# kanyu369/ADNM-UNet

Measured on AMD Instinct MI355X. Metric: sequences/sec training ADNM-UNet 5->20x128x128, higher is better.
Workload: dtype bf16; 1 GPU; ADNM-UNet create_ADNMUNet(5,20,6) 128x128 full training step (fwd + enRainfallLoss + bwd + clip_grad_norm_ + AdamW), recipe parameters, synthetic radar frames in HBM; per_gpu_batch=4, global_batch=4, frames=5->20, parallelism=single, launch=hipGraph replay

## Files before the change

### adnm-unet_amd/csrc/adnm_common.h

```cpp
#pragma once
#include <hip/hip_runtime.h>
#include <hip/hip_bf16.h>
#include <stdint.h>
#include <stdio.h>
#include <stdarg.h>
#include <string.h>
#include "../../include/adnm_hip.h"

#define ADNM_WAVE 64

void adnm_set_error(const char* fmt, ...);

struct AdnmProfScope {
  AdnmProfScope(const char* name, hipStream_t st, double bytes);
  ~AdnmProfScope();
  hipStream_t st_;
  long idx_;
};
#define ADNM_PROF(name, st, bytes) AdnmProfScope adnm_prof_scope__(name, st, (double)(bytes))

struct AdnmFoldSeg {
  float* ptr;
  int len;
};
void adnm_launch_fold(const char* prof_name, const float* part, int rows, int n, AdnmFoldSeg s0, AdnmFoldSeg s1, AdnmFoldSeg s2,
                      AdnmFoldSeg s3, hipStream_t st);

int64_t adnm_lgemm_ws_bytes(int64_t I, int64_t J, int64_t R, int nbs);
int adnm_lgemm_launch(bool b_oc, const float* a, int64_t lda, const void* b, int64_t ldb, int b_dtype, const float* b_scale, const float* bias, float* c,
                      int64_t ldc, void* ws, int64_t ws_bytes, void* slabs_uc, int64_t slabs_uc_bytes, int64_t I, int64_t J, int64_t R, int nbs, int prec,
                      float* q, const char* prof, double prof_bytes, hipStream_t st);
static inline int64_t adnm_ticket_bytes(int64_t ntiles) { return (ntiles * 4 + 255) / 256 * 256; }

struct AdnmLeaf {
  int kind, grid, prec;
  const char* prof;
  double bytes;
  alignas(16) unsigned char args[200];
};
enum {
  ADNM_LEAF_SKGEMM_TN = 0, ADNM_LEAF_DWCONV_WGRAD_K3 = 1, ADNM_LEAF_DWCONV_WGRAD_K5 = 2, ADNM_LEAF_TSGEMM_TN = 3,
  ADNM_LEAF_DWCONV_WALK3 = 4,
  ADNM_LEAF_CONV3_WGRAD = 5,
  ADNM_LEAF_COLSUM = 6,
  ADNM_LEAF_KINDS = 7
};
bool adnm_leafq_active();
bool adnm_leafq_push(const AdnmLeaf& leaf);
int adnm_skgemm_tn_launch_multi(const AdnmLeaf* const* items, int n, hipStream_t st);
int adnm_dwconv_wgrad_launch_multi(const AdnmLeaf* const* items, int n, int K, hipStream_t st);
int adnm_dwconv_walk3_launch_multi(const AdnmLeaf* const* items, int n, hipStream_t st);
int adnm_conv3_wgrad_launch_multi(const AdnmLeaf* const* items, int n, hipStream_t st);
int adnm_tsgemm_tn_launch_multi(const AdnmLeaf* const* items, int n, hipStream_t st);

constexpr int ADNM_GROUP_MAX = 8;
constexpr int ADNM_GROUP_POS_LAST = 1 << 20;
struct AdnmGroupRec;
typedef int (*AdnmGroupFn)(const AdnmGroupRec* const* recs, int n, hipStream_t st);
struct AdnmGroupRec {
  AdnmGroupFn fn;
  int grid, pos;
  const char* prof;
  double bytes;
  alignas(16) unsigned char args[232];
};
bool adnm_group_open();
void adnm_launch_fold_recorded(const char* prof_name, const float* part, int rows, int n, AdnmFoldSeg s0, AdnmFoldSeg s1, AdnmFoldSeg s2,
                               AdnmFoldSeg s3, hipStream_t st);
int adnm_group_submit(const AdnmGroupRec& rec, hipStream_t st);
template <typename Args>
struct AdnmMulti {
  int blk_end[ADNM_GROUP_MAX];
  Args p[ADNM_GROUP_MAX];
};
template <typename Args>
static inline unsigned adnm_group_pack(const AdnmGroupRec* const* r, int n, AdnmMulti<Args>& m) {
  static_assert(sizeof(Args) <= sizeof(AdnmGroupRec::args), "the argument struct must fit a group record");
  static_assert(sizeof(AdnmMulti<Args>) <= 4096, "the descriptor table must fit the kernel argument segment");
  int blocks = 0;
  for (int k = 0; k < ADNM_GROUP_MAX; ++k) {
    if (k < n) memcpy(&m.p[k], r[k]->args, sizeof(Args)), blocks += r[k]->grid;
    else m.p[k] = m.p[0];
    m.blk_end[k] = blocks;
  }
  return (unsigned)blocks;
}
template <typename M>
__device__ __forceinline__ int adnm_group_which(const M& m, int* bid, int* nblk) {
  int k = 0;
#pragma unroll
  for (int i = 0; i < ADNM_GROUP_MAX - 1; ++i) k += (int)blockIdx.x >= m.blk_end[i] ? 1 : 0;
  const int b0 = k ? m.blk_end[k - 1] : 0;
  *bid = (int)blockIdx.x - b0, *nblk = m.blk_end[k] - b0;
  return k;
}

#define ADNM_REQUIRE(cond, ...)            \
  do {                                     \
    if (!(cond)) {                         \
      adnm_set_error(__VA_ARGS__);         \
      return ADNM_EINVAL;                  \
    }                                      \
  } while (0)

#define ADNM_CHECK_LAUNCH(name)                                              \
  do {                                                                       \
    hipError_t e__ = hipGetLastError();                                      \
    if (e__ != hipSuccess) {                                                 \
      adnm_set_error("%s: launch failed: %s", name, hipGetErrorString(e__)); \
      return ADNM_ELAUNCH;                                                   \
    }                                                                        \
  } while (0)

#include <atomic>
#include <initializer_list>
static inline int adnm_allow_lds(const void* fn, size_t smem, std::atomic<uint64_t>& done, const char* name) {
  if (smem <= 64 * 1024) return ADNM_OK;
  int dev = 0;
  if (hipGetDevice(&dev) != hipSuccess) dev = 0;
  const uint64_t bit = 1ull << (dev & 63);
  if (done.load(std::memory_order_relaxed) & bit) return ADNM_OK;
  const hipError_t e = hipFuncSetAttribute(fn, hipFuncAttributeMaxDynamicSharedMemorySize, 160 * 1024);
  if (e != hipSuccess) {
    adnm_set_error("%s: cannot raise the dynamic LDS limit to %zu bytes on device %d: %s", name, smem, dev, hipGetErrorString(e));
    return ADNM_ELAUNCH;
  }
  done.fetch_or(bit, std::memory_order_relaxed);
  return ADNM_OK;
}
#define ADNM_ALLOW_LDS(kernel, smem, name)                                             \
  do {                                                                                 \
    static std::atomic<uint64_t> lds_done__{0};                                        \
    if (int rc__ = adnm_allow_lds((const void*)(kernel), (smem), lds_done__, name)) return rc__; \
  } while (0)

static inline int64_t adnm_cdiv(int64_t a, int64_t b) { return (a + b - 1) / b; }
static inline bool adnm_quad_aligned(int dtype, std::initializer_list<const void*> ptrs) {
  uintptr_t bits = 0;
  for (const void* p : ptrs) bits |= (uintptr_t)p;
  return bits % (dtype == ADNM_BF16 ? 8 : 16) == 0;
}
static inline int64_t adnm_align(int64_t a, int64_t b) { return adnm_cdiv(a, b) * b; }

struct bf16x4 {
  uint16_t v[4];
};

__device__ __forceinline__ float bf16_to_f32(uint16_t h) { return __uint_as_float(((uint32_t)h) << 16); }
__device__ __forceinline__ uint16_t f32_to_bf16(float f) {
  __hip_bfloat16 b = __float2bfloat16(f);
  return *reinterpret_cast<uint16_t*>(&b);
}

template <typename T>
struct Io;
template <>
struct Io<float> {
  static __device__ __forceinline__ float4 ld4(const float* p) { return *reinterpret_cast<const float4*>(p); }
  static __device__ __forceinline__ void st4(float* p, float4 v) { *reinterpret_cast<float4*>(p) = v; }
  static __device__ __forceinline__ float ld(const float* p) { return *p; }
  static __device__ __forceinline__ void st(float* p, float v) { *p = v; }
  static __device__ __forceinline__ float rt(float v) { return v; }
};
template <>
struct Io<uint16_t> {
  static __device__ __forceinline__ float4 ld4(const uint16_t* p) {
    uint2 r = *reinterpret_cast<const uint2*>(p);
    return make_float4(__uint_as_float(r.x << 16), __uint_as_float(r.x & 0xffff0000u), __uint_as_float(r.y << 16),
                       __uint_as_float(r.y & 0xffff0000u));
  }
  static __device__ __forceinline__ void st4(uint16_t* p, float4 v) {
    uint2 r;
    r.x = (uint32_t)f32_to_bf16(v.x) | ((uint32_t)f32_to_bf16(v.y) << 16);
    r.y = (uint32_t)f32_to_bf16(v.z) | ((uint32_t)f32_to_bf16(v.w) << 16);
    *reinterpret_cast<uint2*>(p) = r;
  }
  static __device__ __forceinline__ float ld(const uint16_t* p) { return bf16_to_f32(*p); }
  static __device__ __forceinline__ void st(uint16_t* p, float v) { *p = f32_to_bf16(v); }
  static __device__ __forceinline__ float rt(float v) { return bf16_to_f32(f32_to_bf16(v)); }
};

template <int BT>
__device__ __forceinline__ float4 adnm_ldb4(const void* base, int64_t off) {
  if constexpr (BT == ADNM_B_BF16) {
    const uint2 r = *reinterpret_cast<const uint2*>(reinterpret_cast<const uint16_t*>(base) + off);
    return make_float4(__uint_as_float(r.x << 16), __uint_as_float(r.x & 0xffff0000u), __uint_as_float(r.y << 16), __uint_as_float(r.y & 0xffff0000u));
  } else if constexpr (BT == ADNM_B_FP8) {
    using f2 = __attribute__((ext_vector_type(2))) float;
    const int r = *reinterpret_cast<const int*>(reinterpret_cast<const uint8_t*>(base) + off);
    const f2 lo = __builtin_amdgcn_cvt_pk_f32_fp8(r, false), hi = __builtin_amdgcn_cvt_pk_f32_fp8(r, true);
    return make_float4(lo[0], lo[1], hi[0], hi[1]);
  } else {
    return *reinterpret_cast<const float4*>(reinterpret_cast<const float*>(base) + off);
  }
}

using adnm_f32x4 = __attribute__((ext_vector_type(4))) float;
using adnm_bf16x8 = __attribute__((ext_vector_type(8))) __bf16;

struct AdnmQuant {
  float scale_a, scale_b, amax_a, amax_b, fmax_a, fmax_b, record, pad;
};

struct AdnmStepStats {
  double applied, skipped, norm_sum, norm_max, last_norm, clip_count, loss_sum, loss_nonfinite;
  int skip;
  float sumsq;
};
__device__ __forceinline__ bool adnm_nonfinite_bits(float v) { return (__float_as_uint(v) & 0x7f800000u) == 0x7f800000u; }

__device__ __forceinline__ adnm_bf16x8 adnm_pack_bf16x8(const float (&v)[8]) {
  using f8 = __attribute__((ext_vector_type(8))) float;
  const f8 t = {v[0], v[1], v[2], v[3], v[4], v[5], v[6], v[7]};
  return __builtin_convertvector(t, adnm_bf16x8);
}
template <bool BF8>
__device__ __forceinline__ long adnm_pack_f8x8(const float (&v)[8]) {
  constexpr float kMax = BF8 ? 57344.f : 448.f;
  float c[8];
#pragma unroll
  for (int i = 0; i < 8; ++i) c[i] = __builtin_amdgcn_fmed3f(v[i], kMax, -kMax);
  int lo = 0, hi = 0;
  if (BF8) {
    lo = __builtin_amdgcn_cvt_pk_bf8_f32(c[0], c[1], lo, false), lo = __builtin_amdgcn_cvt_pk_bf8_f32(c[2], c[3], lo, true);
    hi = __builtin_amdgcn_cvt_pk_bf8_f32(c[4], c[5], hi, false), hi = __builtin_amdgcn_cvt_pk_bf8_f32(c[6], c[7], hi, true);
  } else {
    lo = __builtin_amdgcn_cvt_pk_fp8_f32(c[0], c[1], lo, false), lo = __builtin_amdgcn_cvt_pk_fp8_f32(c[2], c[3], lo, true);
    hi = __builtin_amdgcn_cvt_pk_fp8_f32(c[4], c[5], hi, false), hi = __builtin_amdgcn_cvt_pk_fp8_f32(c[6], c[7], hi, true);
  }
  return (long)(((unsigned long)(unsigned)hi << 32) | (unsigned long)(unsigned)lo);
}
template <int PREC, bool P_BF8 = false, bool Q_BF8 = false>
__device__ __forceinline__ adnm_f32x4 adnm_mfma32(const float (&p)[8], const float (&q)[8], adnm_f32x4 acc) {
  if constexpr (PREC == ADNM_MFMA_BF16) {
    return __builtin_amdgcn_mfma_f32_16x16x32_bf16(adnm_pack_bf16x8(p), adnm_pack_bf16x8(q), acc, 0, 0, 0);
  } else if constexpr (PREC == ADNM_MFMA_FP8) {
    const long a = adnm_pack_f8x8<P_BF8>(p), b = adnm_pack_f8x8<Q_BF8>(q);
    if constexpr (P_BF8 && Q_BF8) return __builtin_amdgcn_mfma_f32_16x16x32_bf8_bf8(a, b, acc, 0, 0, 0);
    else if constexpr (P_BF8) return __builtin_amdgcn_mfma_f32_16x16x32_bf8_fp8(a, b, acc, 0, 0, 0);
    else if constexpr (Q_BF8) return __builtin_amdgcn_mfma_f32_16x16x32_fp8_bf8(a, b, acc, 0, 0, 0);
    else return __builtin_amdgcn_mfma_f32_16x16x32_fp8_fp8(a, b, acc, 0, 0, 0);
  } else {
#pragma unroll
    for (int e = 0; e < 8; ++e) acc = __builtin_amdgcn_mfma_f32_16x16x4f32(p[e], q[e], acc, 0, 0, 0);
    return acc;
  }
}
template <int PREC, bool P_BF8 = false, bool Q_BF8 = false>
__device__ __forceinline__ adnm_f32x4 adnm_mfma16(const float (&p)[4], const float (&q)[4], adnm_f32x4 acc) {
  if constexpr (PREC == ADNM_MFMA_F32) {
#pragma unroll
    for (int e = 0; e < 4; ++e) acc = __builtin_amdgcn_mfma_f32_16x16x4f32(p[e], q[e], acc, 0, 0, 0);
    return acc;
  } else {
    const float p8[8] = {p[0], p[1], p[2], p[3], 0.f, 0.f, 0.f, 0.f}, q8[8] = {q[0], q[1], q[2], q[3], 0.f, 0.f, 0.f, 0.f};
    return adnm_mfma32<PREC, P_BF8, Q_BF8>(p8, q8, acc);
  }
}
template <int PREC>
struct AdnmFrag {
  float v[8];
};
template <>
struct AdnmFrag<ADNM_MFMA_BF16> {
  adnm_bf16x8 v;
};
template <>
struct AdnmFrag<ADNM_MFMA_FP8> {
  long v;
};
template <int PREC, bool BF8>
__device__ __forceinline__ AdnmFrag<PREC> adnm_make_frag(const float (&lo)[4], const float* hi, float scale) {
  AdnmFrag<PREC> f;
  float t[8];
#pragma unroll
  for (int e = 0; e < 4; ++e) t[e] = lo[e], t[4 + e] = hi ? hi[e] : 0.f;
  if constexpr (PREC == ADNM_MFMA_BF16) {
    f.v = adnm_pack_bf16x8(t);
  } else if constexpr (PREC == ADNM_MFMA_FP8) {
#pragma unroll
    for (int e = 0; e < 8; ++e) t[e] *= scale;
    f.v = adnm_pack_f8x8<BF8>(t);
  } else {
#pragma unroll
    for (int e = 0; e < 8; ++e) f.v[e] = t[e];
  }
  return f;
}
template <int PREC, bool P_BF8, bool Q_BF8, bool HALF = false>
__device__ __forceinline__ adnm_f32x4 adnm_mma(const AdnmFrag<PREC>& p, const AdnmFrag<PREC>& q, adnm_f32x4 acc) {
  if constexpr (PREC == ADNM_MFMA_BF16) {
    return __builtin_amdgcn_mfma_f32_16x16x32_bf16(p.v, q.v, acc, 0, 0, 0);
  } else if constexpr (PREC == ADNM_MFMA_FP8) {
    if constexpr (P_BF8 && Q_BF8) return __builtin_amdgcn_mfma_f32_16x16x32_bf8_bf8(p.v, q.v, acc, 0, 0, 0);
    else if constexpr (P_BF8) return __builtin_amdgcn_mfma_f32_16x16x32_bf8_fp8(p.v, q.v, acc, 0, 0, 0);
    else if constexpr (Q_BF8) return __builtin_amdgcn_mfma_f32_16x16x32_fp8_bf8(p.v, q.v, acc, 0, 0, 0);
    else return __builtin_amdgcn_mfma_f32_16x16x32_fp8_fp8(p.v, q.v, acc, 0, 0, 0);
  } else {
#pragma unroll
    for (int e = 0; e < (HALF ? 4 : 8); ++e) acc = __builtin_amdgcn_mfma_f32_16x16x4f32(p.v[e], q.v[e], acc, 0, 0, 0);
    return acc;
  }
}

__device__ __forceinline__ float adnm_amax4(float m, float a, float b, float c, float d) {
  return fmaxf(fmaxf(m, fmaxf(fabsf(a), fabsf(b))), fmaxf(fabsf(c), fabsf(d)));
}
__device__ __forceinline__ void adnm_amax_commit(float* slot, float m) {
#pragma unroll
  for (int o = 32; o >= 1; o >>= 1) m = fmaxf(m, __shfl_xor(m, o, 64));
  if ((threadIdx.x & 63) == 0 && m > 0.f) atomicMax(reinterpret_cast<unsigned int*>(slot), __float_as_uint(m));
}

__device__ __forceinline__ float sigmoidf_(float x) { return 1.0f / (1.0f + __expf(-x)); }
__device__ __forceinline__ float siluf_(float x) { return x * sigmoidf_(x); }
__device__ __forceinline__ float silu_gradf_(float x) {
  float s = sigmoidf_(x);
  return s * (1.0f + x * (1.0f - s));
}
__device__ __forceinline__ float geluf_(float x) { return 0.5f * x * (1.0f + erff(x * 0.70710678118654752f)); }
__device__ __forceinline__ float gelu_gradf_(float x) {
  return 0.5f * (1.0f + erff(x * 0.70710678118654752f)) + x * 0.39894228040143268f * __expf(-0.5f * x * x);
}
__device__ __forceinline__ float softplusf_(float x) {
  if (x > 20.0f) return x;
  const float e = __expf(x);
  if (e < 0.25f) {
    const float p = fmaf(e, fmaf(e, fmaf(e, fmaf(e, fmaf(e, fmaf(e, fmaf(e, -0.125f, 1.0f / 7.0f), -1.0f / 6.0f), 0.2f), -0.25f), 1.0f / 3.0f), -0.5f), 1.0f);
    return e * p;
  }
  return __logf(1.0f + e);
}

template <bool GRAD>
__device__ __forceinline__ float adnm_rainloss_term(float p, float t, float omega, float alpha, float gamma, float* g) {
  const float diff = p - t;
  const bool over = p >= t, heavy = t >= 0.7f;
  const float w = over ? 1.0f - omega : omega;
  const float wi = heavy ? alpha * __expf(t) : 0.f;
  float e = w * fabsf(diff) * (1.0f + wi);
  if (GRAD) *g = w * (1.0f + wi) * (diff > 0.f ? 1.f : (diff < 0.f ? -1.f : 0.f));
  if (gamma != 0.f && heavy && !over) {
    const float ex = __expf(alpha * (t - p));
    e += gamma * (ex - 1.0f);
    if (GRAD) *g -= gamma * alpha * ex;
  }
  return e;
}

__device__ __forceinline__ float eval_scaled(float v, float value_scale) { return fminf(fmaxf(v, 0.f), 1.f) * value_scale; }
__device__ __forceinline__ float eval_trunc(float scaled) { return floorf(scaled); }

template <int ACT>
__device__ __forceinline__ float act_fwd(float x) {
  if (ACT == ADNM_ACT_SILU) return siluf_(x);
  if (ACT == ADNM_ACT_GELU) return geluf_(x);
  return x;
}
template <int ACT>
__device__ __forceinline__ float act_grad(float x) {
  if (ACT == ADNM_ACT_SILU) return silu_gradf_(x);
  if (ACT == ADNM_ACT_GELU) return gelu_gradf_(x);
  return 1.0f;
}

__device__ __forceinline__ float wave_sum_from(float v, int lo) {
#pragma unroll
  for (int o = 32; o >= 1; o >>= 1)
    if (o >= lo) v += __shfl_xor(v, o, 64);
  return v;
}
__device__ __forceinline__ float wave_sum(float v) { return wave_sum_from(v, 1); }
__device__ __forceinline__ float group_sum(float v, int width) {
#pragma unroll
  for (int o = 32; o >= 1; o >>= 1)
    if (o < width) v += __shfl_xor(v, o, 64);
  return v;
}
```

### adnm-unet_amd/csrc/lgemm.hip

```cpp
#include "adnm_common.h"

namespace {

using f32x4 = adnm_f32x4;
constexpr int kThreads = 256, kTile = 64, kStep = 32;

template <int PREC>
struct Geo {
  static constexpr bool BF16 = PREC == ADNM_MFMA_BF16, FP8 = PREC == ADNM_MFMA_FP8;
  static constexpr int rc_stride = FP8 ? 10 : (BF16 ? 24 : 40);
  static constexpr int rc_words = kTile * rc_stride;
  static constexpr int oc_stride = 68;
  static constexpr int oc_rows = BF16 ? kStep / 2 : kStep;
  static constexpr int oc_words = FP8 ? rc_words : oc_rows * oc_stride;
};

struct LgArgs {
  const float* A;
  int64_t lda;
  const void* B;
  int64_t ldb;
  const float* b_scale;
  const float* bias;
  float* C;
  int64_t ldc;
  float* slab;
  int* tickets;
  int uc;
  int I, J, R;
  int tiles_j, nbs, kt_per_slice, nkt;
  AdnmQuant* q;
};

__device__ __forceinline__ float4 keep_if(bool ok, float4 v) { return make_float4(ok ? v.x : 0.f, ok ? v.y : 0.f, ok ? v.z : 0.f, ok ? v.w : 0.f); }
__device__ __forceinline__ uint32_t pack2(float lo, float hi) {
  using bf2 = __attribute__((ext_vector_type(2))) __bf16;
  using f2 = __attribute__((ext_vector_type(2))) float;
  const f2 v = {lo, hi};
  return __builtin_bit_cast(uint32_t, __builtin_convertvector(v, bf2));
}

template <bool MULTI>
struct LgPick;
template <>
struct LgPick<false> {
  using Arg = LgArgs;
  static __device__ __forceinline__ const LgArgs& get(const LgArgs& a, int*, int*) { return a; }
};
template <>
struct LgPick<true> {
  using Arg = AdnmMulti<LgArgs>;
  static __device__ __forceinline__ const __attribute__((address_space(4))) LgArgs& get(const Arg&, int* bid, int* nblk) {
    const auto& m = *(const __attribute__((address_space(4))) Arg*)__builtin_amdgcn_kernarg_segment_ptr();
    return m.p[adnm_group_which(m, bid, nblk)];
  }
};
template <bool B_OC, int PREC, bool A_BF8, int D, int BT, bool MULTI>
__global__ __launch_bounds__(kThreads) void lgemm_kernel(typename LgPick<MULTI>::Arg arg) {
  int bid_ = 0, nblk_ = 0;
  const auto& p = LgPick<MULTI>::get(arg, &bid_, &nblk_);
  static_assert(BT == ADNM_B_F32 || (BT == ADNM_B_BF16 && PREC == ADNM_MFMA_BF16) || (BT == ADNM_B_FP8 && PREC == ADNM_MFMA_FP8),
                "a narrow weight shadow feeds the matrix-core precision it was made for");
  constexpr bool BF16 = PREC == ADNM_MFMA_BF16, FP8 = PREC == ADNM_MFMA_FP8;
  using G = Geo<PREC>;
  constexpr int kAW = G::rc_words, kBW = B_OC ? G::oc_words : G::rc_words;
  __shared__ __attribute__((aligned(16))) uint32_t lds[2 * (kAW + kBW)];
  uint32_t* const ldsA = lds;
  uint32_t* const ldsB = lds + 2 * kAW;
  const int tid = threadIdx.x, lane = tid & 63, l15 = lane & 15, kq = lane >> 4;
  const int wave = __builtin_amdgcn_readfirstlane(tid >> 6), wi = wave >> 1, wj = wave & 1;

  int lin = MULTI ? bid_ : (int)blockIdx.x;
  const int nblk = MULTI ? nblk_ : (int)gridDim.x;
  if (MULTI) __builtin_assume(lin >= 0 && nblk > 0 && lin < nblk);
  if ((nblk & 7) == 0) lin = (lin & 7) * (nblk >> 3) + (lin >> 3);
  const int tile = lin / p.nbs, slice = lin - tile * p.nbs;
  const int i0 = (tile / p.tiles_j) * kTile, j0 = (tile % p.tiles_j) * kTile;
  const int kt0 = slice * p.kt_per_slice;
  const int nkt = p.nkt - kt0 < p.kt_per_slice ? p.nkt - kt0 : p.kt_per_slice;

  const int q = tid & 7, lrow = tid >> 3;
  const int cq = tid & 15, lr = tid >> 4;
  const float* a_row[2];
  int b_off[2];
#pragma unroll
  for (int u = 0; u < 2; ++u) {
    const int ia = i0 + lrow + 32 * u;
    a_row[u] = p.A + (int64_t)(ia < p.I ? ia : p.I - 1) * p.lda + 4 * q;
    if (!B_OC) {
      const int jb = j0 + lrow + 32 * u;
      b_off[u] = (int)((int64_t)(jb < p.J ? jb : p.J - 1) * p.ldb + 4 * q);
    } else {
      const int jb = j0 + 4 * cq;
      b_off[u] = (int)((jb + 4 <= p.J ? jb : p.J - 4) + (int64_t)(BF16 ? 2 * lr + u : lr + 16 * u) * p.ldb);
    }
  }
  float4 ra[D][2], rb[D][2];
  auto a_ok = [&](int kt) { return kt < nkt && (kt0 + kt) * kStep + 4 * q < p.R; };
  auto b_ok = [&](int kt, int u) {
    if (!B_OC) return kt < nkt && (kt0 + kt) * kStep + 4 * q < p.R;
    return kt < nkt && (kt0 + kt) * kStep + (BF16 ? 2 * lr + u : lr + 16 * u) < p.R;
  };
  int a_dead[2];
#pragma unroll
  for (int u = 0; u < 2; ++u) a_dead[u] = (int)(p.A - a_row[u]);
  auto load = [&](int kt, float4 (&av)[2], float4 (&bv)[2]) {
    const int r0 = (kt0 + kt) * kStep;
    const bool oka = a_ok(kt);
#pragma unroll
    for (int u = 0; u < 2; ++u) {
      av[u] = *reinterpret_cast<const float4*>(a_row[u] + (oka ? r0 : a_dead[u]));
      const int64_t bo = b_ok(kt, u) ? b_off[u] + (B_OC ? r0 * (int)p.ldb : r0) : 0;
      if constexpr (BT == ADNM_B_FP8)
        bv[u] = make_float4(__int_as_float(*reinterpret_cast<const int*>(reinterpret_cast<const uint8_t*>(p.B) + bo)), 0.f, 0.f, 0.f);
      else bv[u] = adnm_ldb4<BT>(p.B, bo);
    }
  };
  float q_sa = 1.f, q_sb = 1.f, q_sbo = 1.f, amax_a = 0.f, amax_b = 0.f;
  bool rec_a = false, rec_b = false;
  if (p.q) {
    if (PREC == ADNM_MFMA_FP8) q_sa = p.q->scale_a, q_sb = q_sbo = p.q->scale_b;
    const bool rec = p.q->record != 0.f;
    rec_a = rec && (tile % p.tiles_j) == 0, rec_b = BT == ADNM_B_F32 && rec && (tile / p.tiles_j) == 0;
  }
  if (BT == ADNM_B_FP8) q_sb = 1.f, q_sbo = *p.b_scale;
  auto stage = [&](int kt, int buf, const float4 (&av)[2], const float4 (&bv)[2]) {
    uint32_t* const sa = ldsA + buf * kAW;
    uint32_t* const sb = ldsB + buf * kBW;
    const bool oka = a_ok(kt);
    if (rec_a) {
#pragma unroll
      for (int u = 0; u < 2; ++u) {
        const float4 v = keep_if(oka, av[u]);
        amax_a = adnm_amax4(amax_a, v.x, v.y, v.z, v.w);
      }
    }
    if (rec_b) {
#pragma unroll
      for (int u = 0; u < 2; ++u) {
        const float4 v = keep_if(b_ok(kt, u), bv[u]);
        amax_b = adnm_amax4(amax_b, v.x, v.y, v.z, v.w);
      }
    }
    if constexpr (FP8) {
      auto q4 = [](float4 v, float sc, bool bf8) {
        const float c0 = __builtin_amdgcn_fmed3f(v.x * sc, bf8 ? 57344.f : 448.f, bf8 ? -57344.f : -448.f);
        const float c1 = __builtin_amdgcn_fmed3f(v.y * sc, bf8 ? 57344.f : 448.f, bf8 ? -57344.f : -448.f);
        const float c2 = __builtin_amdgcn_fmed3f(v.z * sc, bf8 ? 57344.f : 448.f, bf8 ? -57344.f : -448.f);
        const float c3 = __builtin_amdgcn_fmed3f(v.w * sc, bf8 ? 57344.f : 448.f, bf8 ? -57344.f : -448.f);
        int w = 0;
        if (bf8) w = __builtin_amdgcn_cvt_pk_bf8_f32(c0, c1, w, false), w = __builtin_amdgcn_cvt_pk_bf8_f32(c2, c3, w, true);
        else w = __builtin_amdgcn_cvt_pk_fp8_f32(c0, c1, w, false), w = __builtin_amdgcn_cvt_pk_fp8_f32(c2, c3, w, true);
        return (uint32_t)w;
      };
#pragma unroll
      for (int u = 0; u < 2; ++u) sa[(lrow + 32 * u) * G::rc_stride + q] = q4(keep_if(oka, av[u]), q_sa, A_BF8);
#pragma unroll
      for (int u = 0; u < 2; ++u) {
        const float4 v = keep_if(b_ok(kt, u), bv[u]);
        const uint32_t w = BT == ADNM_B_FP8 ? (uint32_t)__float_as_int(v.x) : q4(v, q_sb, false);
        if (!B_OC) {
          sb[(lrow + 32 * u) * G::rc_stride + q] = w;
        } else {
          uint8_t* const sb8 = reinterpret_cast<uint8_t*>(sb);
          const int k = lr + 16 * u;
#pragma unroll
          for (int c = 0; c < 4; ++c) sb8[(4 * cq + c) * (4 * G::rc_stride) + k] = (uint8_t)(w >> (8 * c));
        }
      }
      return;
    }
#pragma unroll
    for (int u = 0; u < 2; ++u) {
      const float4 v = keep_if(oka, av[u]);
      uint32_t* dst = sa + (lrow + 32 * u) * G::rc_stride;
      if (BF16) *reinterpret_cast<uint2*>(dst + 2 * q) = make_uint2(pack2(v.x, v.y), pack2(v.z, v.w));
      else *reinterpret_cast<float4*>(dst + 4 * q) = v;
    }
    if (!B_OC) {
#pragma unroll
      for (int u = 0; u < 2; ++u) {
        const float4 v = keep_if(b_ok(kt, u), bv[u]);
        uint32_t* dst = sb + (lrow + 32 * u) * G::rc_stride;
        if (BF16) *reinterpret_cast<uint2*>(dst + 2 * q) = make_uint2(pack2(v.x, v.y), pack2(v.z, v.w));
        else *reinterpret_cast<float4*>(dst + 4 * q) = v;
      }
    } else if (BF16) {
      const float4 v0 = keep_if(b_ok(kt, 0), bv[0]), v1 = keep_if(b_ok(kt, 1), bv[1]);
      *reinterpret_cast<uint4*>(sb + lr * G::oc_stride + 4 * cq) = make_uint4(pack2(v0.x, v1.x), pack2(v0.y, v1.y), pack2(v0.z, v1.z), pack2(v0.w, v1.w));
    } else {
#pragma unroll
      for (int u = 0; u < 2; ++u) *reinterpret_cast<float4*>(sb + (lr + 16 * u) * G::oc_stride + 4 * cq) = keep_if(b_ok(kt, u), bv[u]);
    }
  };

  f32x4 acc[2][2];
#pragma unroll
  for (int a = 0; a < 2; ++a)
#pragma unroll
    for (int b = 0; b < 2; ++b) acc[a][b] = f32x4{0.f, 0.f, 0.f, 0.f};

  auto compute = [&](int buf) {
    const uint32_t* const sa = ldsA + buf * kAW;
    const uint32_t* const sb = ldsB + buf * kBW;
    if constexpr (FP8) {
      AdnmFrag<ADNM_MFMA_FP8> fa[2], fb[2];
#pragma unroll
      for (int a = 0; a < 2; ++a) fa[a].v = *reinterpret_cast<const long*>(sa + (32 * wi + 16 * a + l15) * G::rc_stride + 2 * kq);
#pragma unroll
      for (int b = 0; b < 2; ++b) fb[b].v = *reinterpret_cast<const long*>(sb + (32 * wj + 16 * b + l15) * G::rc_stride + 2 * kq);
#pragma unroll
      for (int a = 0; a < 2; ++a)
#pragma unroll
        for (int b = 0; b < 2; ++b) acc[a][b] = adnm_mma<ADNM_MFMA_FP8, false, A_BF8>(fb[b], fa[a], acc[a][b]);
    } else if constexpr (BF16) {
      uint4 fa[2], fb[2];
#pragma unroll
      for (int a = 0; a < 2; ++a) fa[a] = *reinterpret_cast<const uint4*>(sa + (32 * wi + 16 * a + l15) * G::rc_stride + 4 * kq);
#pragma unroll
      for (int b = 0; b < 2; ++b) {
        if (!B_OC) fb[b] = *reinterpret_cast<const uint4*>(sb + (32 * wj + 16 * b + l15) * G::rc_stride + 4 * kq);
        else {
          const uint32_t* s = sb + (4 * kq) * G::oc_stride + 32 * wj + 16 * b + l15;
          fb[b] = make_uint4(s[0], s[G::oc_stride], s[2 * G::oc_stride], s[3 * G::oc_stride]);
        }
      }
#pragma unroll
      for (int a = 0; a < 2; ++a)
#pragma unroll
        for (int b = 0; b < 2; ++b)
          acc[a][b] = __builtin_amdgcn_mfma_f32_16x16x32_bf16(__builtin_bit_cast(adnm_bf16x8, fb[b]), __builtin_bit_cast(adnm_bf16x8, fa[a]), acc[a][b], 0, 0, 0);
    } else {
      float fa[2][2][4], fb[2][2][4];
#pragma unroll
      for (int g = 0; g < 2; ++g) {
#pragma unroll
        for (int a = 0; a < 2; ++a) {
          const float4 v = *reinterpret_cast<const float4*>(sa + (32 * wi + 16 * a + l15) * G::rc_stride + 16 * g + 4 * kq);
          fa[a][g][0] = v.x, fa[a][g][1] = v.y, fa[a][g][2] = v.z, fa[a][g][3] = v.w;
        }
#pragma unroll
        for (int b = 0; b < 2; ++b) {
          if (!B_OC) {
            const float4 v = *reinterpret_cast<const float4*>(sb + (32 * wj + 16 * b + l15) * G::rc_stride + 16 * g + 4 * kq);
            fb[b][g][0] = v.x, fb[b][g][1] = v.y, fb[b][g][2] = v.z, fb[b][g][3] = v.w;
          } else {
            const float* s = reinterpret_cast<const float*>(sb) + (16 * g + 4 * kq) * G::oc_stride + 32 * wj + 16 * b + l15;
#pragma unroll
            for (int e = 0; e < 4; ++e) fb[b][g][e] = s[e * G::oc_stride];
          }
        }
      }
      AdnmFrag<PREC> pa[2], pb[2];
#pragma unroll
      for (int a = 0; a < 2; ++a) pa[a] = adnm_make_frag<PREC, A_BF8>(fa[a][0], fa[a][1], q_sa);
#pragma unroll
      for (int b = 0; b < 2; ++b) pb[b] = adnm_make_frag<PREC, false>(fb[b][0], fb[b][1], q_sb);
#pragma unroll
      for (int a = 0; a < 2; ++a)
#pragma unroll
        for (int b = 0; b < 2; ++b) acc[a][b] = adnm_mma<PREC, false, A_BF8>(pb[b], pa[a], acc[a][b]);
    }
  };

#pragma unroll
  for (int s = 0; s < D; ++s) {
    load(s, ra[s], rb[s]);
    __builtin_amdgcn_sched_barrier(0);
  }
  for (int t = 0; t < nkt; t += D) {
#pragma unroll
    for (int s = 0; s < D; ++s) {
      stage(t + s, s & 1, ra[s], rb[s]);
      load(t + s + D, ra[s], rb[s]);
      __syncthreads();
      compute(s & 1);
      __builtin_amdgcn_sched_barrier(0);
    }
  }

  if (rec_a) adnm_amax_commit(&p.q->amax_a, amax_a);
  if (rec_b) adnm_amax_commit(&p.q->amax_b, amax_b);
  if (PREC == ADNM_MFMA_FP8) {
    const float inv = 1.0f / (q_sa * q_sbo);
#pragma unroll
    for (int a = 0; a < 2; ++a)
#pragma unroll
      for (int b = 0; b < 2; ++b) acc[a][b] = acc[a][b] * inv;
  }
  const bool split = p.nbs > 1;
  float* const slab = split ? p.slab + ((int64_t)tile * p.nbs + slice) * (kTile * kTile) : nullptr;
  const bool vec_ok = (p.ldc & 3) == 0 && (p.J & 3) == 0 && (reinterpret_cast<uintptr_t>(p.C) & 15) == 0 &&
                      (!p.bias || (reinterpret_cast<uintptr_t>(p.bias) & 15) == 0);
#pragma unroll
  for (int a = 0; a < 2; ++a) {
    const int il = 32 * wi + 16 * a + l15;
#pragma unroll
    for (int b = 0; b < 2; ++b) {
      const int jl = 32 * wj + 16 * b + 4 * kq;
      const f32x4 v = acc[a][b];
      if (split) {
        *reinterpret_cast<float4*>(slab + il * kTile + jl) = make_float4(v[0], v[1], v[2], v[3]);
      } else if (i0 + il < p.I) {
        const int jg = j0 + jl;
        float* dst = p.C + (int64_t)(i0 + il) * p.ldc + jg;
        if (vec_ok && jg + 3 < p.J) {
          float4 bv = make_float4(0.f, 0.f, 0.f, 0.f);
          if (p.bias) bv = *reinterpret_cast<const float4*>(p.bias + jg);
          *reinterpret_cast<float4*>(dst) = make_float4(v[0] + bv.x, v[1] + bv.y, v[2] + bv.z, v[3] + bv.w);
        } else {
#pragma unroll
          for (int r = 0; r < 4; ++r)
            if (jg + r < p.J) dst[r] = v[r] + (p.bias ? p.bias[jg + r] : 0.f);
        }
      }
    }
  }
  if (!split) return;

  asm volatile("s_waitcnt vmcnt(0)" ::: "memory");
  __syncthreads();
  int* const flag = reinterpret_cast<int*>(lds);
  if (tid == 0) {
    if (!p.uc) {
      __builtin_amdgcn_fence(__ATOMIC_RELEASE, "agent");
      asm volatile("s_waitcnt vmcnt(0)" ::: "memory");
    }
    const int drawn = __hip_atomic_fetch_add(p.tickets + tile, 1, __ATOMIC_RELAXED, __HIP_MEMORY_SCOPE_AGENT);
    if (drawn == p.nbs - 1) {
      if (!p.uc) {
        __builtin_amdgcn_fence(__ATOMIC_ACQUIRE, "agent");
        asm volatile("s_waitcnt vmcnt(0)" ::: "memory");
      }
      __hip_atomic_store(p.tickets + tile, 0, __ATOMIC_RELAXED, __HIP_MEMORY_SCOPE_AGENT);
    }
    *flag = drawn;
  }
  __syncthreads();
  if (*flag != p.nbs - 1) return;
  {
    const int il = tid >> 2, jl = (tid & 3) * 16;
    const int ig = i0 + il, jg = j0 + jl;
    if (ig >= p.I || jg >= p.J) return;
    const float* src = p.slab + (int64_t)tile * p.nbs * (kTile * kTile) + il * kTile + jl;
    float4 sum[4];
#pragma unroll
    for (int c = 0; c < 4; ++c) sum[c] = make_float4(0.f, 0.f, 0.f, 0.f);
#pragma unroll 2
    for (int s = 0; s < p.nbs; ++s) {
      float4 v[4];
#pragma unroll
      for (int c = 0; c < 4; ++c) v[c] = *reinterpret_cast<const float4*>(src + (int64_t)s * (kTile * kTile) + 4 * c);
#pragma unroll
      for (int c = 0; c < 4; ++c) sum[c].x += v[c].x, sum[c].y += v[c].y, sum[c].z += v[c].z, sum[c].w += v[c].w;
    }
    float* dst = p.C + (int64_t)ig * p.ldc + jg;
#pragma unroll
    for (int c = 0; c < 4; ++c) {
      if (jg + 4 * c >= p.J) break;
      float4 o = sum[c];
      if (p.bias) {
        const float* bp = p.bias + jg + 4 * c;
        o.x += bp[0], o.y += bp[1], o.z += bp[2], o.w += bp[3];
      }
      *reinterpret_cast<float4*>(dst + 4 * c) = o;
    }
  }
}

constexpr int kRingDepth = 4;

template <bool B_OC, int PREC, bool A_BF8, int BT>
int lg_group_fn(const AdnmGroupRec* const* r, int n, hipStream_t st) {
  if (n == 1) {
    LgArgs p;
    memcpy(&p, r[0]->args, sizeof(LgArgs));
    lgemm_kernel<B_OC, PREC, A_BF8, kRingDepth, BT, false><<<(unsigned)r[0]->grid, kThreads, 0, st>>>(p);
    return ADNM_OK;
  }
  AdnmMulti<LgArgs> m;
  const unsigned blocks = adnm_group_pack(r, n, m);
  lgemm_kernel<B_OC, PREC, A_BF8, kRingDepth, BT, true><<<blocks, kThreads, 0, st>>>(m);
  return ADNM_OK;
}

struct LgPlan {
  int tiles_i, tiles_j, ntiles, nkt, nbs, kt_per_slice;
};
LgPlan make_plan(int64_t I, int64_t J, int64_t R, int nbs) {
  LgPlan pl;
  pl.tiles_i = (int)adnm_cdiv(I, kTile);
  pl.tiles_j = (int)adnm_cdiv(J, kTile);
  pl.ntiles = pl.tiles_i * pl.tiles_j;
  pl.nkt = (int)adnm_cdiv(R, kStep);
  if (nbs > pl.nkt) nbs = pl.nkt;
  if (nbs > 32) nbs = 32;
  if (nbs < 1 || J % 4 != 0) nbs = 1;
  pl.kt_per_slice = (int)adnm_cdiv(pl.nkt, nbs);
  pl.nbs = (int)adnm_cdiv(pl.nkt, pl.kt_per_slice);
  return pl;
}
}

int64_t adnm_lgemm_ws_bytes(int64_t I, int64_t J, int64_t R, int nbs) {
  const LgPlan pl = make_plan(I, J, R, nbs);
  return pl.nbs > 1 ? adnm_ticket_bytes(pl.ntiles) + (int64_t)pl.ntiles * pl.nbs * kTile * kTile * (int64_t)sizeof(float) : 16;
}

int adnm_lgemm_launch(bool b_oc, const float* a, int64_t lda, const void* b, int64_t ldb, int b_dtype, const float* b_scale, const float* bias, float* c,
                      int64_t ldc, void* ws, int64_t ws_bytes, void* slabs_uc, int64_t slabs_uc_bytes, int64_t I, int64_t J, int64_t R, int nbs, int prec,
                      float* q, const char* prof, double prof_bytes, hipStream_t st) {
  const LgPlan pl = make_plan(I, J, R, nbs);
  LgArgs p;
  p.A = a, p.lda = lda, p.B = b, p.ldb = ldb, p.b_scale = b_scale, p.bias = bias, p.C = c, p.ldc = ldc;
  ADNM_REQUIRE(J * ldb < (1ll << 31) && R * ldb < (1ll << 31), "skgemm: weight beyond 2^31 elements (32-bit lane offsets)");
  p.I = (int)I, p.J = (int)J, p.R = (int)R;
  p.tiles_j = pl.tiles_j, p.nbs = pl.nbs, p.kt_per_slice = pl.kt_per_slice, p.nkt = pl.nkt;
  p.slab = nullptr, p.tickets = nullptr, p.uc = 0;
  p.q = reinterpret_cast<AdnmQuant*>(q);
  if (pl.nbs > 1) {
    const int64_t slab_bytes = (int64_t)pl.ntiles * pl.nbs * kTile * kTile * (int64_t)sizeof(float);
    const bool uc = slabs_uc && slabs_uc_bytes >= slab_bytes;
    const int64_t need = uc ? adnm_ticket_bytes(pl.ntiles) : adnm_lgemm_ws_bytes(I, J, R, nbs);
    if (!ws || ws_bytes < need) {
      adnm_set_error("skgemm: workspace %lld < %lld bytes", (long long)ws_bytes, (long long)need);
      return ADNM_EWORKSPACE;
    }
    ADNM_REQUIRE(((uintptr_t)ws & 255) == 0 && ((uintptr_t)slabs_uc & 255) == 0, "skgemm: a split launch needs 256-byte aligned workspaces");
    p.tickets = (int*)ws;
    p.slab = uc ? (float*)slabs_uc : (float*)((char*)ws + adnm_ticket_bytes(pl.ntiles));
    p.uc = uc ? 1 : 0;
  }
  static_assert(sizeof(LgArgs) <= sizeof(AdnmGroupRec::args), "LgArgs must fit a group record");
  AdnmGroupRec rec;
  rec.grid = pl.ntiles * pl.nbs, rec.pos = 0, rec.prof = prof, rec.bytes = prof_bytes;
  memcpy(rec.args, &p, sizeof(LgArgs));
#define LG(OC)                                                                                              \
  do {                                                                                                      \
    if (b_dtype == ADNM_B_BF16) rec.fn = lg_group_fn<OC, ADNM_MFMA_BF16, false, ADNM_B_BF16>;               \
    else if (b_dtype == ADNM_B_FP8 && prec == ADNM_MFMA_FP8) rec.fn = lg_group_fn<OC, ADNM_MFMA_FP8, false, ADNM_B_FP8>; \
    else if (b_dtype == ADNM_B_FP8) rec.fn = lg_group_fn<OC, ADNM_MFMA_FP8, true, ADNM_B_FP8>;              \
    else if (prec == ADNM_MFMA_BF16) rec.fn = lg_group_fn<OC, ADNM_MFMA_BF16, false, ADNM_B_F32>;           \
    else if (prec == ADNM_MFMA_FP8) rec.fn = lg_group_fn<OC, ADNM_MFMA_FP8, false, ADNM_B_F32>;             \
    else if (prec == ADNM_MFMA_FP8_GRAD) rec.fn = lg_group_fn<OC, ADNM_MFMA_FP8, true, ADNM_B_F32>;         \
    else rec.fn = lg_group_fn<OC, ADNM_MFMA_F32, false, ADNM_B_F32>;                                        \
  } while (0)
  if (!b_oc) LG(false);
  else LG(true);
#undef LG
  return adnm_group_submit(rec, st);
}
```

### adnm-unet_amd/csrc/skgemm.hip

```cpp
#include "adnm_common.h"

namespace {

using f32x4 = adnm_f32x4;
constexpr int kBlock = 512;
constexpr int kWaves = kBlock / 64;

struct SkArgs {
  const float* A;
  int64_t sa_i, sa_r;
  const void* B;
  int64_t sb_r, sb_j;
  const float* b_scale;
  const float* bias;
  float* C;
  int64_t ldc, slice_stride;
  float* bsum;
  int64_t bsum_stride;
  int I, J, R;
  int tiles_j, ntiles, nbs, wpt, chunks_per_wave, nchunks;
  int* tickets;
  int uc;
  float* out;
  int64_t ldo;
  AdnmQuant* q;
};

template <bool A_RC, bool B_RC, int PREC, bool A_BF8, int TM, int TN, int KC, int BT = ADNM_B_F32, typename Args>
__device__ __forceinline__ void skgemm_body(const Args& p, const int bid, const int nblk) {
  static_assert(BT == ADNM_B_F32 || (BT == ADNM_B_BF16 && PREC == ADNM_MFMA_BF16) || (BT == ADNM_B_FP8 && PREC == ADNM_MFMA_FP8),
                "a narrow weight shadow feeds the matrix-core precision it was made for");
  static_assert((A_RC || TM == 4) && (B_RC || TN == 4), "an operand contiguous along the output axis is 4 interleaved blocks wide");
  constexpr int kAcc = TM * TN * 256;
  constexpr int kBuf = kAcc + 4 * 64;
  __shared__ __attribute__((aligned(16))) float red[(kWaves / 2) * kBuf];
  const int wave = __builtin_amdgcn_readfirstlane(threadIdx.x >> 6);
  const int gw = wave % p.wpt, group = wave / p.wpt;
  int ts = bid * (kWaves / p.wpt) + group;
  const bool active = ts < p.ntiles * p.nbs;
  int tile, bslice;
  if (p.tickets) {
    if ((nblk & 7) == 0) ts = (bid & 7) * (nblk >> 3) + (bid >> 3);
    tile = ts / p.nbs, bslice = ts % p.nbs;
  } else {
    tile = active ? ts % p.ntiles : 0, bslice = active ? ts / p.ntiles : 0;
  }
  const int i0 = (tile / p.tiles_j) * 16 * TM, j0 = (tile % p.tiles_j) * 16 * TN;
  const int lane = threadIdx.x & 63, l15 = lane & 15, kk = lane >> 4;
  const int c0 = active ? (bslice * p.wpt + gw) * p.chunks_per_wave : 0;
  const int c1 = !active ? 0 : (c0 + p.chunks_per_wave < p.nchunks ? c0 + p.chunks_per_wave : p.nchunks);

  auto fetch = [&](int c, bool live, float (&av)[TM][KC][4], float (&bv)[TN][KC][4]) {
#pragma unroll
    for (int s = 0; s < KC; ++s) {
      const int r0 = (c * KC + s) * 16;
      const int rq4 = r0 + 4 * kk < p.R ? r0 + 4 * kk : 0;
      if constexpr (A_RC) {
#pragma unroll
        for (int t = 0; t < TM; ++t) {
          const int row = i0 + 16 * t + l15, rc = row < p.I ? row : p.I - 1;
          const float4 v = *reinterpret_cast<const float4*>(p.A + (live ? (int64_t)rc * p.sa_i + rq4 : 0));
          av[t][s][0] = v.x, av[t][s][1] = v.y, av[t][s][2] = v.z, av[t][s][3] = v.w;
        }
      } else {
        const int row = i0 + 4 * l15, rc = row < p.I ? row : p.I - 4;
#pragma unroll
        for (int e = 0; e < 4; ++e) {
          const int rr = r0 + 4 * kk + e, rq = rr < p.R ? rr : p.R - 1;
          const float4 v = *reinterpret_cast<const float4*>(p.A + (live ? (int64_t)rq * p.sa_r + rc : 0));
          av[0][s][e] = v.x, av[1 % TM][s][e] = v.y, av[2 % TM][s][e] = v.z, av[3 % TM][s][e] = v.w;
        }
      }
      if constexpr (B_RC) {
#pragma unroll
        for (int t = 0; t < TN; ++t) {
          const int col = j0 + 16 * t + l15, cc = col < p.J ? col : p.J - 1;
          const float4 v = adnm_ldb4<BT>(p.B, live ? (int64_t)cc * p.sb_j + rq4 : 0);
          bv[t][s][0] = v.x, bv[t][s][1] = v.y, bv[t][s][2] = v.z, bv[t][s][3] = v.w;
        }
      } else {
        const int col = j0 + 4 * l15, cc = col < p.J ? col : p.J - 4;
#pragma unroll
        for (int e = 0; e < 4; ++e) {
          const int rr = r0 + 4 * kk + e, rq = rr < p.R ? rr : p.R - 1;
          const float4 v = adnm_ldb4<BT>(p.B, live ? (int64_t)rq * p.sb_r + cc : 0);
          bv[0][s][e] = v.x, bv[1 % TN][s][e] = v.y, bv[2 % TN][s][e] = v.z, bv[3 % TN][s][e] = v.w;
        }
      }
    }
  };

  f32x4 acc[TM][TN];
#pragma unroll
  for (int a = 0; a < TM; ++a)
#pragma unroll
    for (int b = 0; b < TN; ++b) acc[a][b] = f32x4{0.f, 0.f, 0.f, 0.f};
  float bs[4] = {0.f, 0.f, 0.f, 0.f};
  float q_sa = 1.f, q_sb = 1.f, q_sbo = 1.f, amax_a = 0.f, amax_b = 0.f;
  bool rec_a = false, rec_b = false;
  if (p.q) {
    if (PREC == ADNM_MFMA_FP8) q_sa = p.q->scale_a, q_sb = q_sbo = p.q->scale_b;
    const bool rec = p.q->record != 0.f && active;
    rec_a = rec && (tile % p.tiles_j) == 0, rec_b = BT == ADNM_B_F32 && rec && (tile / p.tiles_j) == 0;
  }
  if (BT == ADNM_B_FP8) q_sb = 1.f, q_sbo = *p.b_scale;
  auto compute = [&](int c, float (&av)[TM][KC][4], const float (&bv)[TN][KC][4]) {
#pragma unroll
    for (int s = 0; s < KC; ++s) {
      const int r0 = (c * KC + s) * 16;
      if (r0 + 16 > p.R) {
#pragma unroll
        for (int e = 0; e < 4; ++e)
          if (r0 + 4 * kk + (A_RC ? 0 : e) >= p.R) {
#pragma unroll
            for (int t = 0; t < TM; ++t) av[t][s][e] = 0.f;
          }
      }
      if (!A_RC && p.bsum) {
#pragma unroll
        for (int t = 0; t < TM; ++t) bs[t] += (av[t][s][0] + av[t][s][1]) + (av[t][s][2] + av[t][s][3]);
      }
      if (rec_a) {
#pragma unroll
        for (int t = 0; t < TM; ++t) amax_a = adnm_amax4(amax_a, av[t][s][0], av[t][s][1], av[t][s][2], av[t][s][3]);
      }
      if (rec_b && r0 + 16 <= p.R) {
#pragma unroll
        for (int t = 0; t < TN; ++t) amax_b = adnm_amax4(amax_b, bv[t][s][0], bv[t][s][1], bv[t][s][2], bv[t][s][3]);
      }
    }
#pragma unroll
    for (int s = 0; s < KC; s += 2) {
      constexpr bool kHalf = (KC & 1) != 0;
      AdnmFrag<PREC> fa[TM], fb[TN];
#pragma unroll
      for (int a = 0; a < TM; ++a) fa[a] = adnm_make_frag<PREC, A_BF8>(av[a][s], kHalf ? nullptr : av[a][(s + 1) % KC], q_sa);
#pragma unroll
      for (int b = 0; b < TN; ++b) fb[b] = adnm_make_frag<PREC, false>(bv[b][s], kHalf ? nullptr : bv[b][(s + 1) % KC], q_sb);
#pragma unroll
      for (int a = 0; a < TM; ++a)
#pragma unroll
        for (int b = 0; b < TN; ++b) {
          if (B_RC) acc[a][b] = adnm_mma<PREC, false, A_BF8, kHalf>(fb[b], fa[a], acc[a][b]);
          else acc[a][b] = adnm_mma<PREC, A_BF8, false, kHalf>(fa[a], fb[b], acc[a][b]);
        }
    }
  };
  float a0[TM][KC][4], b0[TN][KC][4], a1[TM][KC][4], b1[TN][KC][4], a2[TM][KC][4], b2[TN][KC][4];
  const int cl = c1 > c0 ? c1 - 1 : 0;
  auto fetch_at = [&](int c, float (&av)[TM][KC][4], float (&bv)[TN][KC][4]) { fetch(c < c1 ? c : cl, c < c1, av, bv); };
  fetch_at(c0, a0, b0);
  __builtin_amdgcn_sched_barrier(0);
  fetch_at(c0 + 1, a1, b1);
  __builtin_amdgcn_sched_barrier(0);
  for (int c = c0; c < c1; c += 3) {
    fetch_at(c + 2, a2, b2);
    __builtin_amdgcn_sched_barrier(0);
    compute(c, a0, b0);
    __builtin_amdgcn_sched_barrier(0);
    fetch_at(c + 3, a0, b0);
    __builtin_amdgcn_sched_barrier(0);
    if (c + 1 < c1) compute(c + 1, a1, b1);
    __builtin_amdgcn_sched_barrier(0);
    fetch_at(c + 4, a1, b1);
    __builtin_amdgcn_sched_barrier(0);
    if (c + 2 < c1) compute(c + 2, a2, b2);
    __builtin_amdgcn_sched_barrier(0);
  }

  if (rec_a) adnm_amax_commit(&p.q->amax_a, amax_a);
  if (rec_b) adnm_amax_commit(&p.q->amax_b, amax_b);
  if (PREC == ADNM_MFMA_FP8) {
    const float inv = 1.0f / (q_sa * q_sbo);
#pragma unroll
    for (int a = 0; a < TM; ++a)
#pragma unroll
      for (int b = 0; b < TN; ++b) acc[a][b] = acc[a][b] * inv;
  }
  for (int half = p.wpt >> 1; half >= 1; half >>= 1) {
    if (gw >= half && gw < 2 * half) {
      float* buf = red + (group * (p.wpt >> 1) + (gw - half)) * kBuf;
#pragma unroll
      for (int a = 0; a < TM; ++a)
#pragma unroll
        for (int b = 0; b < TN; ++b)
#pragma unroll
          for (int r = 0; r < 4; ++r) buf[((a * TN + b) * 4 + r) * 64 + lane] = acc[a][b][r];
      if (!A_RC) {
#pragma unroll
        for (int t = 0; t < 4; ++t) buf[kAcc + t * 64 + lane] = bs[t];
      }
    }
    __syncthreads();
    if (gw < half) {
      const float* buf = red + (group * (p.wpt >> 1) + gw) * kBuf;
#pragma unroll
      for (int a = 0; a < TM; ++a)
#pragma unroll
        for (int b = 0; b < TN; ++b)
#pragma unroll
          for (int r = 0; r < 4; ++r) acc[a][b][r] += buf[((a * TN + b) * 4 + r) * 64 + lane];
      if (!A_RC) {
#pragma unroll
        for (int t = 0; t < 4; ++t) bs[t] += buf[kAcc + t * 64 + lane];
      }
    }
    __syncthreads();
  }
  if (!p.tickets && (!active || gw != 0)) return;

  if (gw == 0) {
    float* Cp = p.C + (int64_t)bslice * p.slice_stride;
    const bool add_bias = p.bias && bslice == 0 && !p.tickets;
    if constexpr (B_RC) {
      const bool vec_ok = (p.ldc & 3) == 0 && (reinterpret_cast<uintptr_t>(Cp) & 15) == 0 && (!add_bias || (reinterpret_cast<uintptr_t>(p.bias) & 15) == 0);
#pragma unroll
      for (int a = 0; a < TM; ++a) {
        const int ig = i0 + 16 * a + l15;
        if (ig >= p.I) continue;
#pragma unroll
        for (int b = 0; b < TN; ++b) {
          const int jg = j0 + 16 * b + 4 * kk;
          if (vec_ok && jg + 3 < p.J) {
            float4 bv4 = make_float4(0.f, 0.f, 0.f, 0.f);
            if (add_bias) bv4 = *reinterpret_cast<const float4*>(p.bias + jg);
            *reinterpret_cast<float4*>(Cp + (int64_t)ig * p.ldc + jg) =
                make_float4(acc[a][b][0] + bv4.x, acc[a][b][1] + bv4.y, acc[a][b][2] + bv4.z, acc[a][b][3] + bv4.w);
          } else {
#pragma unroll
            for (int r = 0; r < 4; ++r)
              if (jg + r < p.J) Cp[(int64_t)ig * p.ldc + jg + r] = acc[a][b][r] + (add_bias ? p.bias[jg + r] : 0.f);
          }
        }
      }
    } else {
#pragma unroll
      for (int a = 0; a < TM; ++a)
#pragma unroll
        for (int r = 0; r < 4; ++r) {
          const int il = kk * 4 + r;
          const int ig = A_RC ? i0 + 16 * a + il : i0 + 4 * il + a;
          if (ig >= p.I) continue;
          const int jg = j0 + 4 * l15;
          if (jg < p.J)
            *reinterpret_cast<float4*>(Cp + (int64_t)ig * p.ldc + jg) = make_float4(acc[a][0][r], acc[a][1 % TN][r], acc[a][2 % TN][r], acc[a][3 % TN][r]);
        }
    }
    if (!A_RC && p.bsum && (tile % p.tiles_j) == 0) {
#pragma unroll
      for (int t = 0; t < 4; ++t) bs[t] += __shfl_xor(bs[t], 16, 64), bs[t] += __shfl_xor(bs[t], 32, 64);
      const int ig = i0 + 4 * l15;
      if (kk == 0 && ig < p.I) *reinterpret_cast<float4*>(p.bsum + (int64_t)bslice * p.bsum_stride + ig) = make_float4(bs[0], bs[1], bs[2], bs[3]);
    }
  }
  if (!p.tickets) return;

  int* flag = reinterpret_cast<int*>(red);
  if (wave == 0) {
    asm volatile("s_waitcnt vmcnt(0)" ::: "memory");
    if (lane == 0) {
      if (!p.uc) {
        __builtin_amdgcn_fence(__ATOMIC_RELEASE, "agent");
        asm volatile("s_waitcnt vmcnt(0)" ::: "memory");
      }
      const int drawn = __hip_atomic_fetch_add(p.tickets + tile, 1, __ATOMIC_RELAXED, __HIP_MEMORY_SCOPE_AGENT);
      if (drawn == p.nbs - 1) {
        if (!p.uc) {
          __builtin_amdgcn_fence(__ATOMIC_ACQUIRE, "agent");
          asm volatile("s_waitcnt vmcnt(0)" ::: "memory");
        }
        __hip_atomic_store(p.tickets + tile, 0, __ATOMIC_RELAXED, __HIP_MEMORY_SCOPE_AGENT);
      }
      *flag = drawn;
    }
  }
  __syncthreads();
  if (*flag != p.nbs - 1) return;
  {
    constexpr int kQuads = 4 * TN;
    const int jg = j0 + 4 * (threadIdx.x % kQuads);
    if (jg >= p.J) return;
    for (int il = threadIdx.x / kQuads; il < 16 * TM; il += kBlock / kQuads) {
      const int ig = i0 + il;
      if (ig >= p.I) break;
      const float* src = p.C + (int64_t)ig * p.ldc + jg;
      float4 sum = make_float4(0.f, 0.f, 0.f, 0.f);
#pragma unroll 4
      for (int s = 0; s < p.nbs; ++s) {
        const float4 u = *reinterpret_cast<const float4*>(src + (int64_t)s * p.slice_stride);
        sum.x += u.x, sum.y += u.y, sum.z += u.z, sum.w += u.w;
      }
      if (p.bias) sum.x += p.bias[jg], sum.y += p.bias[jg + 1], sum.z += p.bias[jg + 2], sum.w += p.bias[jg + 3];
      *reinterpret_cast<float4*>(p.out + (int64_t)ig * p.ldo + jg) = sum;
    }
  }
}

template <bool A_RC, bool B_RC, int PREC, bool A_BF8, int TM, int TN, int KC, int BT>
__global__ __launch_bounds__(kBlock) void skgemm_kernel(SkArgs p) {
  skgemm_body<A_RC, B_RC, PREC, A_BF8, TM, TN, KC, BT>(p, (int)blockIdx.x, (int)gridDim.x);
}

template <bool A_RC, bool B_RC, int PREC, bool A_BF8, int TM, int TN, int KC, int BT>
__global__ __launch_bounds__(kBlock) void skgemm_multi_kernel(AdnmMulti<SkArgs> by_value) {
  (void)by_value;
  const auto& m = *(const __attribute__((address_space(4))) AdnmMulti<SkArgs>*)__builtin_amdgcn_kernarg_segment_ptr();
  int bid, nblk;
  const int k = adnm_group_which(m, &bid, &nblk);
  skgemm_body<A_RC, B_RC, PREC, A_BF8, TM, TN, KC, BT>(m.p[k], bid, nblk);
}

constexpr int kMaxSk = 16;
struct MultiSk {
  int count, blk_end[kMaxSk];
  SkArgs p[kMaxSk];
};
static_assert(sizeof(MultiSk) <= 4096, "the descriptor table must fit the kernel argument segment");
template <int PREC>
__global__ __launch_bounds__(kBlock) void skgemm_tn_multi_kernel(MultiSk by_value) {
  (void)by_value;
  const auto& m = *(const __attribute__((address_space(4))) MultiSk*)__builtin_amdgcn_kernarg_segment_ptr();
  int k = 0;
  while (k + 1 < m.count && (int)blockIdx.x >= m.blk_end[k]) ++k;
  const int b0 = k ? m.blk_end[k - 1] : 0;
  skgemm_body<false, false, PREC, false, 4, 4, 1>(m.p[k], (int)blockIdx.x - b0, m.blk_end[k] - b0);
}

enum { KERNEL_STREAM = 0, KERNEL_LDS = 1 };
struct Plan {
  int kernel;
  int tm, tn, kc;
  int tiles_i, tiles_j, ntiles, nchunks, wpt, nbs, cpw;
  bool combine;
};

void finish(Plan& pl, int64_t I, int64_t J, int64_t R) {
  pl.tiles_i = (int)adnm_cdiv(I, 16 * pl.tm);
  pl.tiles_j = (int)adnm_cdiv(J, 16 * pl.tn);
  pl.ntiles = pl.tiles_i * pl.tiles_j;
  pl.nchunks = (int)adnm_cdiv(R, 16 * pl.kc);
}
void slice(Plan& pl) {
  if (pl.nbs < 1) pl.nbs = 1;
  pl.cpw = (int)adnm_cdiv(pl.nchunks, pl.nbs * pl.wpt);
  pl.nbs = (int)adnm_cdiv(adnm_cdiv(pl.nchunks, pl.cpw), pl.wpt);
}

struct Forced {
  bool on = false;
  int v[6] = {0, 0, 0, 0, 0, 0};
  Forced() {
    const char* e = getenv("ADNM_SK_FORCE");
    on = e && sscanf(e, "%d,%d,%d,%d,%d,%d", &v[0], &v[1], &v[2], &v[3], &v[4], &v[5]) == 6;
  }
};
const Forced& forced() {
  static const Forced f;
  return f;
}
int use_table() {
  static const int v = [] {
    const char* e = getenv("ADNM_SK_TABLE");
    return e && e[0] == '0' ? 0 : 1;
  }();
  return v;
}
bool config_ok(int op, const Plan& pl) {
  if (pl.kernel == KERNEL_LDS) return op != ADNM_SKGEMM_TN;
  if (pl.kernel != KERNEL_STREAM || pl.wpt < 1 || pl.wpt > kWaves || (pl.wpt & (pl.wpt - 1))) return false;
  const int tm = pl.tm, tn = pl.tn, kc = pl.kc;
  if (op == ADNM_SKGEMM_NT) return (tm == 1 && tn == 1 && kc == 4) || (tm == 2 && tn == 2 && kc == 2) || (tm == 4 && tn == 4 && kc == 1);
  if (op == ADNM_SKGEMM_NN) return tn == 4 && ((tm == 1 && kc == 2) || (tm == 2 && kc == 2) || (tm == 4 && kc == 1));
  return tm == 4 && tn == 4 && kc == 1;
}

struct Tuned {
  int op, I, J, R, bf16;
  int cfg[6];
};
const Tuned kTuned[] = {
#include "skgemm_tuned.inc"
};
const Tuned* tuned(int op, int64_t I, int64_t J, int64_t R, bool bf16) {
  for (const Tuned& t : kTuned)
    if (t.op == op && t.I == I && t.J == J && t.R == R && t.bf16 == (int)bf16) return &t;
  return nullptr;
}
Plan plan_deferred(int64_t I, int64_t J, int64_t R, bool direct, bool bf16) {
  Plan pl;
  pl.kernel = KERNEL_STREAM, pl.combine = false, pl.tm = pl.tn = 4, pl.kc = 1;
  finish(pl, I, J, R);
  const bool force = forced().on;
  const Tuned* tu = force || use_table() == 0 ? nullptr : tuned(ADNM_SKGEMM_TN, I, J, R, bf16);
  if (force || tu) {
    const int* v = force ? forced().v : tu->cfg;
    pl.wpt = v[4], pl.nbs = v[5];
    if (v[0] != KERNEL_STREAM || v[1] != 4 || v[2] != 4 || v[3] != 1 || pl.wpt < 1 || pl.wpt > kWaves || (pl.wpt & (pl.wpt - 1))) {
      pl.kernel = -1;
      return pl;
    }
    while (pl.wpt > 1 && pl.wpt > pl.nchunks) pl.wpt >>= 1;
  } else {
    static const int grouped_waves = [] {
      const char* e = getenv("ADNM_SK_TN_WAVES");
      const int v = e ? atoi(e) : 0;
      return v > 0 ? v : 256;
    }();
    int want = (int)adnm_cdiv(adnm_leafq_active() ? grouped_waves : 2048, pl.ntiles);
    if (want > pl.nchunks) want = pl.nchunks;
    if (want < 1) want = 1;
    pl.wpt = 1;
    while (pl.wpt * 2 <= want && pl.wpt < kWaves) pl.wpt *= 2;
    pl.nbs = (int)adnm_cdiv(want, pl.wpt);
  }
  if (!force && !tu) {
    const int64_t by_mem = (int64_t)(2 << 20) / (I * J * 4);
    if (pl.nbs > by_mem) pl.nbs = (int)by_mem;
  }
  if (pl.nbs > 64) pl.nbs = 64;
  if (pl.nbs < 1 || direct) pl.nbs = 1;
  slice(pl);
  return pl;
}
Plan plan_critical(int op, int64_t I, int64_t J, int64_t R, bool can_split, bool bf16) {
  Plan pl;
  pl.combine = false;
  const bool force = forced().on;
  const Tuned* tu = force || use_table() == 0 ? nullptr : tuned(op, I, J, R, bf16);
  if (force || tu) {
    const int* v = force ? forced().v : tu->cfg;
    pl.kernel = v[0], pl.tm = v[1], pl.tn = v[2], pl.kc = v[3], pl.wpt = v[4], pl.nbs = v[5];
    if (!config_ok(op, pl)) pl.kernel = -1;
  } else {
    const int64_t t64 = adnm_cdiv(I, 64) * adnm_cdiv(J, 64);
    pl.nbs = 1, pl.wpt = kWaves;
    if (op == ADNM_SKGEMM_NT) {
      pl.kernel = (t64 >= 128 || R <= 128 || (R >= 1024 && t64 >= 8)) ? KERNEL_LDS : KERNEL_STREAM;
      if (pl.kernel == KERNEL_LDS && R >= 1024 && t64 <= 128) {
        int want = (int)(192 / t64);
        while (pl.nbs * 2 <= want && pl.nbs < 8) pl.nbs *= 2;
      }
      pl.tm = pl.tn = 2, pl.kc = 2;
      if (adnm_cdiv(I, 32) * adnm_cdiv(J, 32) < 128) pl.tm = pl.tn = 1, pl.kc = 4;
    } else {
      pl.kernel = (t64 >= 256 || R <= 128) ? KERNEL_LDS : KERNEL_STREAM;
      pl.tn = 4, pl.kc = 2, pl.tm = (I >= 256 && t64 >= 100) ? 2 : 1;
    }
  }
  if (pl.kernel != KERNEL_STREAM) {
    if (!can_split || pl.nbs < 1) pl.nbs = 1;
    return pl;
  }
  finish(pl, I, J, R);
  while (pl.wpt > 1 && pl.wpt > pl.nchunks) pl.wpt >>= 1;
  if (!can_split || pl.wpt != kWaves) pl.nbs = 1;
  if (pl.nbs > 32) pl.nbs = 32;
  slice(pl);
  pl.combine = pl.nbs > 1;
  return pl;
}
Plan make_plan(int op, int64_t I, int64_t J, int64_t R, bool direct, bool bf16) {
  return op == ADNM_SKGEMM_TN ? plan_deferred(I, J, R, direct, bf16) : plan_critical(op, I, J, R, !direct && J % 4 == 0, bf16);
}

}

namespace {
int shape_ok(int op, int64_t M, int64_t N, int64_t K) {
  if (M < 1 || N < 4 || K < 4 || M > (1 << 20) || N > 16384 || K > 16384 || M * N >= (1ll << 31) || M * K >= (1ll << 31)) return 0;
  if (op == ADNM_SKGEMM_NT) return K % 4 == 0;
  if (op == ADNM_SKGEMM_NN) return N % 4 == 0 && K % 4 == 0;
  if (op == ADNM_SKGEMM_TN) return N % 4 == 0 && K % 4 == 0;
  return 0;
}
void dims(int op, int64_t M, int64_t N, int64_t K, int64_t* I, int64_t* J, int64_t* R) {
  if (op == ADNM_SKGEMM_NT) *I = M, *J = N, *R = K;
  else if (op == ADNM_SKGEMM_NN) *I = M, *J = K, *R = N;
  else *I = N, *J = K, *R = M;
}

template <bool A_RC, bool B_RC, int PREC, bool A_BF8, int TM, int TN, int KC, int BT>
int sk_group_fn(const AdnmGroupRec* const* r, int n, hipStream_t st) {
  if constexpr (A_RC) {
    if (n > 1) {
      AdnmMulti<SkArgs> m;
      const unsigned blocks = adnm_group_pack(r, n, m);
      skgemm_multi_kernel<A_RC, B_RC, PREC, A_BF8, TM, TN, KC, BT><<<blocks, kBlock, 0, st>>>(m);
      return ADNM_OK;
    }
  }
  for (int k = 0; k < n; ++k) {
    SkArgs p;
    memcpy(&p, r[k]->args, sizeof(SkArgs));
    skgemm_kernel<A_RC, B_RC, PREC, A_BF8, TM, TN, KC, BT><<<(unsigned)r[k]->grid, kBlock, 0, st>>>(p);
  }
  return ADNM_OK;
}
template <bool A_RC, bool B_RC, int TM, int TN, int KC>
AdnmGroupFn pick(int prec, int bt) {
  if (bt == ADNM_B_BF16) return sk_group_fn<A_RC, B_RC, ADNM_MFMA_BF16, false, TM, TN, KC, ADNM_B_BF16>;
  if (bt == ADNM_B_FP8 && prec == ADNM_MFMA_FP8) return sk_group_fn<A_RC, B_RC, ADNM_MFMA_FP8, false, TM, TN, KC, ADNM_B_FP8>;
  if (bt == ADNM_B_FP8) return sk_group_fn<A_RC, B_RC, ADNM_MFMA_FP8, true, TM, TN, KC, ADNM_B_FP8>;
  if (prec == ADNM_MFMA_BF16) return sk_group_fn<A_RC, B_RC, ADNM_MFMA_BF16, false, TM, TN, KC, ADNM_B_F32>;
  if (prec == ADNM_MFMA_FP8) return sk_group_fn<A_RC, B_RC, ADNM_MFMA_FP8, false, TM, TN, KC, ADNM_B_F32>;
  if (prec == ADNM_MFMA_FP8_GRAD) return sk_group_fn<A_RC, B_RC, ADNM_MFMA_FP8, true, TM, TN, KC, ADNM_B_F32>;
  return sk_group_fn<A_RC, B_RC, ADNM_MFMA_F32, false, TM, TN, KC, ADNM_B_F32>;
}
}

extern "C" int adnm_skgemm_supported(int op, int64_t M, int64_t N, int64_t K) { return shape_ok(op, M, N, K); }

namespace {
int64_t ws_need(const Plan& pl, int64_t I, int64_t J, int64_t R) {
  if (pl.kernel == KERNEL_LDS) return adnm_lgemm_ws_bytes(I, J, R, pl.nbs);
  if (pl.kernel < 0) return 16;
  if (pl.nbs <= 1) return 16;
  return (pl.combine ? adnm_ticket_bytes(pl.ntiles) : 0) + (int64_t)pl.nbs * (I * J + I) * (int64_t)sizeof(float);
}
}

extern "C" int64_t adnm_skgemm_ws_bytes(int op, int64_t M, int64_t N, int64_t K) {
  if (!shape_ok(op, M, N, K)) return -1;
  int64_t I, J, R;
  dims(op, M, N, K, &I, &J, &R);
  const int64_t a = ws_need(make_plan(op, I, J, R, false, false), I, J, R), b = ws_need(make_plan(op, I, J, R, false, true), I, J, R);
  return a > b ? a : b;
}

extern "C" int64_t adnm_skgemm_counter_bytes(int op, int64_t M, int64_t N, int64_t K) {
  if (!shape_ok(op, M, N, K)) return -1;
  if (op == ADNM_SKGEMM_TN) return 0;
  int64_t I, J, R, need = 0;
  dims(op, M, N, K, &I, &J, &R);
  for (int bf = 0; bf < 2; ++bf) {
    const Plan pl = make_plan(op, I, J, R, false, bf != 0);
    if (pl.kernel < 0) continue;
    int64_t ntiles = pl.ntiles, nbs = pl.nbs;
    if (pl.kernel == KERNEL_LDS) {
      ntiles = adnm_cdiv(I, 64) * adnm_cdiv(J, 64);
      nbs = adnm_lgemm_ws_bytes(I, J, R, pl.nbs) > 16 ? 2 : 1;
    }
    if (nbs > 1 && adnm_ticket_bytes(ntiles) > need) need = adnm_ticket_bytes(ntiles);
  }
  return need;
}

extern "C" int adnm_skgemm(int op, const float* a, int64_t lda, const void* b, int64_t ldb, int b_dtype, const float* b_scale, const float* bias,
                           float* c, int64_t ldc, float* dbias, void* ws, int64_t ws_bytes, void* slabs_uc, int64_t slabs_uc_bytes, int64_t M, int64_t N, int64_t K, int prec, float* q,
                           adnm_stream_t stream) {
  ADNM_REQUIRE(prec >= ADNM_MFMA_F32 && prec <= ADNM_MFMA_FP8_GRAD, "skgemm: bad prec %d", prec);
  const bool fp8 = prec == ADNM_MFMA_FP8 || prec == ADNM_MFMA_FP8_GRAD;
  ADNM_REQUIRE(!fp8 || q, "skgemm: the fp8 modes need a quantisation record");
  if (fp8 && op == ADNM_SKGEMM_TN) prec = ADNM_MFMA_BF16, q = nullptr;
  ADNM_REQUIRE(a && b && c, "skgemm: null pointer");
  ADNM_REQUIRE(b_dtype == ADNM_B_F32 || (op != ADNM_SKGEMM_TN && ((b_dtype == ADNM_B_BF16 && prec == ADNM_MFMA_BF16) || (b_dtype == ADNM_B_FP8 && fp8 && b_scale))),
               "skgemm: a narrow weight operand (b_dtype %d) needs op NT / NN and the matching prec (bf16 shadow: ADNM_MFMA_BF16; fp8 shadow: an fp8 mode "
               "and its scale), got op %d prec %d", b_dtype, op, prec);
  ADNM_REQUIRE(shape_ok(op, M, N, K), "skgemm: unsupported op/shape op=%d M=%lld N=%lld K=%lld", op, (long long)M, (long long)N, (long long)K);
  int64_t I, J, R;
  dims(op, M, N, K, &I, &J, &R);
  ADNM_REQUIRE(ldc >= J && ldc % 4 == 0, "skgemm: bad output row stride");
  ADNM_REQUIRE(lda % 4 == 0 && ldb % 4 == 0 && lda >= (op == ADNM_SKGEMM_NT ? K : N) && ldb >= K, "skgemm: bad operand row strides");
  ADNM_REQUIRE(!(bias && op != ADNM_SKGEMM_NT) && !(dbias && op != ADNM_SKGEMM_TN), "skgemm: bias only with NT, dbias only with TN");
  ADNM_REQUIRE(((uintptr_t)a | (uintptr_t)c) % 16 == 0 && (uintptr_t)b % (b_dtype == ADNM_B_F32 ? 16 : (b_dtype == ADNM_B_BF16 ? 8 : 4)) == 0,
               "skgemm: operands must be aligned to 4 elements (16 bytes of fp32)");
  hipStream_t st = (hipStream_t)stream;
  const bool bf = prec != ADNM_MFMA_F32;
  Plan pl = make_plan(op, I, J, R, false, bf);
  if (op == ADNM_SKGEMM_TN && ldc != J) pl = make_plan(op, I, J, R, true, bf);
  ADNM_REQUIRE(pl.kernel >= 0, "skgemm: ADNM_SK_FORCE names a configuration this op has no kernel for");
  if (!(slabs_uc && op != ADNM_SKGEMM_TN)) {
    const int64_t asked = adnm_skgemm_ws_bytes(op, M, N, K);
    if (asked > 16 && (!ws || ws_bytes < asked)) {
      adnm_set_error("skgemm: workspace %lld < %lld bytes", (long long)ws_bytes, (long long)asked);
      return ADNM_EWORKSPACE;
    }
  }
  const char* scope = op == ADNM_SKGEMM_NT ? "skgemm_nt" : (op == ADNM_SKGEMM_NN ? "skgemm_nn" : "skgemm_tn");
  const double algo_bytes = 4.0 * (double)M * (K + N) + (b_dtype == ADNM_B_BF16 ? 2.0 : (b_dtype == ADNM_B_FP8 ? 1.0 : 4.0)) * (double)N * K;
  if (pl.kernel == KERNEL_LDS) {
    const int rc = adnm_lgemm_launch(op == ADNM_SKGEMM_NN, a, lda, b, ldb, b_dtype, b_scale, bias, c, ldc, ws, ws_bytes, slabs_uc, slabs_uc_bytes, I, J, R, pl.nbs, prec, q,
                                     scope, algo_bytes, st);
    if (rc != ADNM_OK) return rc;
    ADNM_CHECK_LAUNCH("skgemm");
    return ADNM_OK;
  }
  const bool split = pl.nbs > 1;
  const int64_t slab_bytes = split ? (int64_t)pl.nbs * (I * J + (dbias ? I : 0)) * (int64_t)sizeof(float) : 0;
  const bool uc = split && pl.combine && slabs_uc && slabs_uc_bytes >= slab_bytes;
  const int64_t need = !split ? 0 : (uc ? adnm_ticket_bytes(pl.ntiles) : ws_need(pl, I, J, R));
  if (split && (!ws || ws_bytes < need)) {
    adnm_set_error("skgemm: workspace %lld < %lld bytes", (long long)ws_bytes, (long long)need);
    return ADNM_EWORKSPACE;
  }
  SkArgs p;
  p.A = a, p.B = b, p.bias = bias, p.b_scale = b_scale;
  if (op == ADNM_SKGEMM_NT) p.sa_i = lda, p.sa_r = 1, p.sb_r = 1, p.sb_j = ldb;
  else if (op == ADNM_SKGEMM_NN) p.sa_i = lda, p.sa_r = 1, p.sb_r = ldb, p.sb_j = 1;
  else p.sa_i = 1, p.sa_r = lda, p.sb_r = ldb, p.sb_j = 1;
  p.I = (int)I, p.J = (int)J, p.R = (int)R;
  p.tiles_j = pl.tiles_j, p.ntiles = pl.ntiles, p.nbs = pl.nbs, p.wpt = pl.wpt, p.chunks_per_wave = pl.cpw, p.nchunks = pl.nchunks;
  float* part = (float*)ws;
  p.C = split ? part : c;
  p.ldc = split ? J : ldc;
  const int64_t rowlen = I * J + (dbias ? I : 0);
  p.slice_stride = split ? rowlen : 0;
  p.bsum = dbias ? (split ? part + I * J : dbias) : nullptr;
  p.bsum_stride = split ? rowlen : 0;
  p.tickets = nullptr, p.out = c, p.ldo = ldc, p.uc = 0;
  p.q = reinterpret_cast<AdnmQuant*>(q);
  if (pl.combine) {
    ADNM_REQUIRE(((uintptr_t)ws & 255) == 0 && ((uintptr_t)slabs_uc & 255) == 0, "skgemm: a split launch needs 256-byte aligned workspaces");
    p.tickets = (int*)ws;
    p.C = uc ? (float*)slabs_uc : (float*)((char*)ws + adnm_ticket_bytes(pl.ntiles));
    p.uc = uc ? 1 : 0;
  }
  const unsigned grid = (unsigned)adnm_cdiv((int64_t)pl.ntiles * pl.nbs, kWaves / pl.wpt);
  bool queued = false;
  if (op == ADNM_SKGEMM_TN && (prec == ADNM_MFMA_F32 || prec == ADNM_MFMA_BF16)) {
    static_assert(sizeof(SkArgs) <= sizeof(AdnmLeaf::args), "SkArgs must fit a leaf record");
    AdnmLeaf leaf;
    leaf.kind = ADNM_LEAF_SKGEMM_TN, leaf.grid = (int)grid, leaf.prec = prec, leaf.prof = scope, leaf.bytes = algo_bytes;
    memcpy(leaf.args, &p, sizeof(SkArgs));
    queued = adnm_leafq_push(leaf);
  }
  if (!queued) {
    static_assert(sizeof(SkArgs) <= sizeof(AdnmGroupRec::args), "SkArgs must fit a group record");
    AdnmGroupRec rec;
    rec.grid = (int)grid, rec.pos = 0, rec.prof = scope, rec.bytes = algo_bytes;
    memcpy(rec.args, &p, sizeof(SkArgs));
    if (op == ADNM_SKGEMM_NT) {
      if (pl.tm == 1) rec.fn = pick<true, true, 1, 1, 4>(prec, b_dtype);
      else if (pl.tm == 2) rec.fn = pick<true, true, 2, 2, 2>(prec, b_dtype);
      else rec.fn = pick<true, true, 4, 4, 1>(prec, b_dtype);
    } else if (op == ADNM_SKGEMM_NN) {
      if (pl.tm == 1) rec.fn = pick<true, false, 1, 4, 2>(prec, b_dtype);
      else if (pl.tm == 2) rec.fn = pick<true, false, 2, 4, 2>(prec, b_dtype);
      else rec.fn = pick<true, false, 4, 4, 1>(prec, b_dtype);
    } else {
      rec.fn = pick<false, false, 4, 4, 1>(prec, b_dtype);
    }
    if (op == ADNM_SKGEMM_TN) {
      const AdnmGroupRec* one = &rec;
      ADNM_PROF(scope, st, algo_bytes);
      rec.fn(&one, 1, st);
    } else if (int rc = adnm_group_submit(rec, st)) {
      return rc;
    }
  }
  ADNM_CHECK_LAUNCH("skgemm");
  if (split && !pl.combine) {
    adnm_launch_fold("skgemm_fold", part, pl.nbs, (int)rowlen, {c, (int)(I * J)}, {dbias, dbias ? (int)I : 0}, {nullptr, 0}, {nullptr, 0}, st);
    ADNM_CHECK_LAUNCH("skgemm_fold");
  }
  return ADNM_OK;
}


int adnm_skgemm_tn_launch_multi(const AdnmLeaf* const* items, int n, hipStream_t st) {
  for (int prec = ADNM_MFMA_F32; prec <= ADNM_MFMA_BF16; ++prec) {
    int i = 0;
    while (i < n) {
      MultiSk m;
      m.count = 0;
      int blocks = 0;
      double bytes = 0;
      for (; i < n && m.count < kMaxSk; ++i) {
        if (items[i]->prec != prec) continue;
        memcpy(&m.p[m.count], items[i]->args, sizeof(SkArgs));
        blocks += items[i]->grid;
        m.blk_end[m.count++] = blocks;
        bytes += items[i]->bytes;
      }
      if (!m.count) break;
      for (int k = m.count; k < kMaxSk; ++k) m.blk_end[k] = blocks;
      ADNM_PROF("skgemm_tn", st, bytes);
      if (prec == ADNM_MFMA_BF16) skgemm_tn_multi_kernel<ADNM_MFMA_BF16><<<(unsigned)blocks, kBlock, 0, st>>>(m);
      else skgemm_tn_multi_kernel<ADNM_MFMA_F32><<<(unsigned)blocks, kBlock, 0, st>>>(m);
    }
  }
  ADNM_CHECK_LAUNCH("skgemm_tn (grouped)");
  return ADNM_OK;
}
```

### include/adnm_hip.h

```cpp
#ifndef ADNM_HIP_H
#define ADNM_HIP_H

#include <stdint.h>
#include <stddef.h>

#ifdef __cplusplus
extern "C" {
#endif

typedef void* adnm_stream_t;

enum { ADNM_F32 = 0, ADNM_BF16 = 1 };
enum { ADNM_ACT_NONE = 0, ADNM_ACT_SILU = 1, ADNM_ACT_GELU = 2 };
enum { ADNM_OK = 0, ADNM_EINVAL = -1, ADNM_ELAUNCH = -2, ADNM_EWORKSPACE = -3 };
enum { ADNM_MFMA_F32 = 0, ADNM_MFMA_BF16 = 1, ADNM_MFMA_FP8 = 2, ADNM_MFMA_FP8_GRAD = 3 };
enum { ADNM_B_F32 = 0, ADNM_B_BF16 = 1, ADNM_B_FP8 = 2 };

int adnm_quant_update(float* table, int64_t n, float* state, float headroom, adnm_stream_t stream);
int adnm_quant_update_guarded(float* table, int64_t n, float* state, float headroom, const void* stats, adnm_stream_t stream);

const char* adnm_last_error(void);
int adnm_abi_version(void);

int adnm_prof_enable(int on);
int64_t adnm_prof_collect(char* buf, int64_t buflen);

void* adnm_foldq_create(void);
int adnm_foldq_destroy(void* q);
int adnm_foldq_bind(void* q);
int64_t adnm_foldq_pending(void* q);
int adnm_foldq_flush(void* q, adnm_stream_t stream);
int adnm_foldq_clear(void* q);
int adnm_foldq_accumulate_next(int mask);

void* adnm_leafq_create(void);
int adnm_leafq_destroy(void* q);
int adnm_leafq_bind(void* q);
int64_t adnm_leafq_pending(void* q);
int adnm_leafq_flush(void* q, adnm_stream_t stream);
int adnm_leafq_clear(void* q);

int adnm_group_begin(void);
int adnm_group_launch(adnm_stream_t stream);
int adnm_group_clear(void);
int64_t adnm_group_pending(void);

int adnm_rownorm_fwd(const void* x, int64_t ldx, const float* w, const float* b, const float* scale,
                     const float* shift, void* y, int64_t ldy, float* mu, float* rstd, int64_t M, int64_t d,
                     float eps, int subtract_mean, int dtype, adnm_stream_t stream);
int64_t adnm_rownorm_bwd_ws_bytes(int64_t M, int64_t d);
int adnm_rownorm_bwd(const void* dy, int64_t lddy, const void* x, int64_t ldx, const float* w, const float* b,
                     const float* scale, const float* mu, const float* rstd, void* dx, int64_t lddx, float* dw,
                     float* db, float* dscale, float* dshift, const void* dres, int64_t lddres, void* ws, int64_t ws_bytes,
                     int64_t M, int64_t d, int subtract_mean, int dtype, adnm_stream_t stream);

int64_t adnm_ssd_ws_bytes(int64_t B, int64_t L, int64_t H, int64_t P, int64_t N, int64_t G);
int adnm_ssd_reduce_fwd(const void* x, int64_t ldx, const void* Bm, int64_t ldb, const void* Cm, int64_t ldc,
                        const void* dt_raw, int64_t lddt, int64_t dt_hstride, const float* dt_bias,
                        const float* A_log, const float* D, int64_t p_hstride, void* y, int64_t ldy, float* kv,
                        const float* ln_w, const float* ln_b, void* yn, int64_t ldyn, float* ln_mu, float* ln_rstd,
                        float ln_eps, void* ws, int64_t ws_bytes, int64_t B, int64_t L, int64_t H, int64_t P, int64_t N,
                        int64_t G, int dtype, adnm_stream_t stream);
int adnm_ssd_reduce_bwd(const void* dy, int64_t lddy, const void* x, int64_t ldx, const void* Bm, int64_t ldb,
                        const void* Cm, int64_t ldc, const void* dt_raw, int64_t lddt, int64_t dt_hstride,
                        const float* dt_bias, const float* A_log, const float* D, int64_t p_hstride,
                        const float* kv, void* dx, int64_t lddx, void* dBm, int64_t lddb, void* dCm, int64_t lddc,
                        void* ddt_raw, int64_t ldddt, float* ddt_bias, float* dA_log, float* dD, void* ws,
                        int64_t ws_bytes, int64_t B, int64_t L, int64_t H, int64_t P, int64_t N, int64_t G,
                        int dtype, adnm_stream_t stream);

int64_t adnm_ssd_scan_ws_bytes(int64_t B, int64_t L, int64_t H, int64_t N, int64_t chunk, int backward);
int adnm_ssd_scan_fwd(const void* x, int64_t ldx, int64_t x_hstride, const void* Bm, int64_t ldb, const void* Cm,
                      int64_t ldc, const void* dt_raw, int64_t lddt, int64_t dt_hstride, const float* dt_bias,
                      const float* A_log, const float* D, int64_t p_hstride, void* y, int64_t ldy, int64_t y_hstride,
                      float* S_in, void* ws, int64_t ws_bytes, int64_t B, int64_t L, int64_t H, int64_t P, int64_t N,
                      int64_t G, int64_t chunk, int reverse, int dtype, adnm_stream_t stream);
int adnm_ssd_scan_bwd(const void* dy, int64_t lddy, int64_t dy_hstride, const void* x, int64_t ldx, int64_t x_hstride,
                      const void* Bm, int64_t ldb, const void* Cm, int64_t ldc, const void* dt_raw, int64_t lddt,
                      int64_t dt_hstride, const float* dt_bias, const float* A_log, const float* D, int64_t p_hstride,
                      const float* S_in, void* dx, int64_t lddx, int64_t dx_hstride, void* dBm, int64_t lddb, void* dCm,
                      int64_t lddc, void* ddt_raw, int64_t ldddt, int64_t ddt_hstride, float* ddt_bias, float* dA_log,
                      float* dD, void* ws, int64_t ws_bytes, int64_t B, int64_t L, int64_t H, int64_t P, int64_t N,
                      int64_t G, int64_t chunk, int reverse, int dtype, adnm_stream_t stream);

int adnm_dwconv_fwd(const void* x, int64_t ldx, const float* wgt, const float* bias, const void* addend,
                    int64_t ldadd, void* y, int64_t ldy, int64_t B, int64_t H, int64_t W, int64_t C, int KH,
                    int KW, int act, int wlayout, int dtype, adnm_stream_t stream);
int64_t adnm_dwconv_bwd_ws_bytes(int64_t B, int64_t H, int64_t W, int64_t C, int KH, int KW);
int adnm_dwconv_bwd(const void* dy, int64_t lddy, const void* x, int64_t ldx, const float* wgt,
                    const float* bias, void* dpre, void* dx, int64_t lddx, float* dwgt, float* dbias, void* ws,
                    int64_t ws_bytes, int64_t B, int64_t H, int64_t W, int64_t C, int KH, int KW, int act,
                    int wlayout, int dtype, adnm_stream_t stream);
int adnm_dwconv_wgrad(const void* g, int64_t ldg, const void* x, int64_t ldx, float* dwgt, float* dbias, void* ws, int64_t ws_bytes,
                      int64_t B, int64_t H, int64_t W, int64_t C, int KH, int KW, int wlayout, int dtype, adnm_stream_t stream);

int adnm_haar_dwt(const void* x, int64_t ldx, int64_t cx, void* y, int64_t B, int64_t H, int64_t W, int64_t C,
                  int dtype, adnm_stream_t stream);
int adnm_wt_level(const float* x, int64_t ldx, int64_t cx, const float* taps, float* sub, float* tag, int64_t B, int64_t H, int64_t W,
                  int64_t C, int K, int flip, adnm_stream_t stream);
int adnm_wt_level_base(const float* x, int64_t ldx, const float* taps, const float* base_taps, const float* base_bias, float* sub, float* tag,
                       float* ybase, int64_t B, int64_t H, int64_t W, int64_t C, int K, int flip, adnm_stream_t stream);
int adnm_haar_idwt(const void* s, const void* up1, const void* up2, const void* ll_add, const void* y_add1, const void* y_add2, void* y,
                   int64_t B, int64_t H, int64_t W, int64_t C, int dtype, adnm_stream_t stream);

int adnm_maxpool_fwd(const void* x, void* y, int64_t B, int64_t H, int64_t W, int64_t C, int kh, int kw, int stride,
                     int dtype, adnm_stream_t stream);
int adnm_maxpool_bwd(const void* dy, const void* x, const void* dx_add, void* dx, int64_t B, int64_t H, int64_t W, int64_t C, int kh,
                     int kw, int stride, int dtype, adnm_stream_t stream);

int64_t adnm_instnorm_ws_bytes(int64_t B, int64_t HW, int64_t C);
int adnm_instnorm_fwd(const void* x, const float* scale, const float* shift, void* y, float* mu, float* rstd,
                      void* ws, int64_t ws_bytes, int64_t B, int64_t HW, int64_t C, float eps, int act, int dtype,
                      adnm_stream_t stream);
int adnm_instnorm_bwd(const void* dy, const void* x, const float* scale, const float* shift, const float* mu,
                      const float* rstd, void* dx, float* dscale, float* dshift, void* ws, int64_t ws_bytes,
                      int64_t B, int64_t HW, int64_t C, int act, int dtype, adnm_stream_t stream);

int64_t adnm_groupnorm_ws_bytes(int64_t B, int64_t HW, int64_t C, int64_t G);
int adnm_groupnorm_fwd(const void* x, const float* gamma, const float* beta, const float* scale, const float* shift, void* y,
                       float* mu, float* rstd, void* ws, int64_t ws_bytes, int64_t B, int64_t HW, int64_t C, int64_t G, float eps,
                       int act, int dtype, adnm_stream_t stream);
int adnm_groupnorm_bwd(const void* dy, const void* x, const float* gamma, const float* beta, const float* scale, const float* shift,
                       const float* mu, const float* rstd, void* dx, float* dgamma, float* dbeta, float* dscale, float* dshift,
                       void* ws, int64_t ws_bytes, int64_t B, int64_t HW, int64_t C, int64_t G, int act, int dtype,
                       adnm_stream_t stream);

int adnm_gate_fwd(const void* h, int64_t ldh, void* y, int64_t ldy, int64_t M, int64_t F, int dtype,
                  adnm_stream_t stream);
int adnm_gate_bwd(const void* dy, int64_t lddy, const void* h, int64_t ldh, void* dh, int64_t lddh, int64_t M,
                  int64_t F, int dtype, adnm_stream_t stream);

int adnm_igate_fwd(const void* x, const float* enhance, const float* threshold, void* y, int64_t n, int dtype,
                   adnm_stream_t stream);
int64_t adnm_igate_bwd_ws_bytes(int64_t n);
int adnm_igate_bwd(const void* dy, const void* x, const float* enhance, const float* threshold, void* dx, float* denhance,
                   float* dthreshold, void* ws, int64_t ws_bytes, int64_t n, int dtype, adnm_stream_t stream);
int adnm_igate_res_fwd(const float* x, const float* res, int per_token, const float* gama, const float* enhance,
                       const float* threshold, float* y, int64_t B, int64_t L, int64_t C, adnm_stream_t stream);
int64_t adnm_igate_res_bwd_ws_bytes(int64_t B, int64_t L, int64_t C);
int adnm_igate_res_bwd(const float* dy, const float* x, const float* res, int per_token, const float* gama, const float* enhance,
                       const float* threshold, float* dx, float* dres, float* dgama, float* denhance, float* dthreshold, void* ws,
                       int64_t ws_bytes, int64_t B, int64_t L, int64_t C, adnm_stream_t stream);


int adnm_skipgate_fwd(const float* x, const float* const* params, float* pooled, float* conv, float* out, int64_t B, int64_t H, int64_t W,
                      int64_t C, adnm_stream_t stream);
int64_t adnm_skipgate_grad_floats(int64_t C);
int64_t adnm_skipgate_bwd_ws_bytes(int64_t B, int64_t H, int64_t W, int64_t C);
int adnm_skipgate_bwd(const float* dout, const float* x, const float* const* params, const float* pooled, const float* conv, float* dx,
                      float* dparams, void* ws, int64_t ws_bytes, int64_t B, int64_t H, int64_t W, int64_t C, adnm_stream_t stream);

int adnm_attn4_fwd(const float* qkv, float* out, float* lse, int64_t B, int64_t L, int64_t heads, float scale, adnm_stream_t stream);
int adnm_attn4_bwd(const float* dout, const float* qkv, const float* out, const float* lse, float* dqkv, int64_t B, int64_t L, int64_t heads,
                   float scale, adnm_stream_t stream);

int adnm_emul_fwd(const float* a, int64_t lda, const float* b, int64_t ldb, float* y, int64_t M, int64_t C, adnm_stream_t stream);
int adnm_emul_bwd(const float* dy, const float* a, int64_t lda, const float* b, int64_t ldb, float* da, float* db, int64_t M, int64_t C,
                  adnm_stream_t stream);
int adnm_chancopy(const float* x, int64_t ldx, int64_t Cin, float* y, int64_t Cout, int64_t M, adnm_stream_t stream);
int adnm_conv1d3_fwd(const float* x, const float* w, const float* bias, float* y, int64_t B, int64_t n, adnm_stream_t stream);
int adnm_conv1d3_bwd(const float* dy, const float* x, const float* w, float* dx, float* dwb, int64_t B, int64_t n, adnm_stream_t stream);
int adnm_bridge_heads_fwd(const float* att, const float* const* W, const float* const* bias, const int64_t* C, int nheads,
                          const float* enhance, const float* threshold, float* const* z, float* const* y, int64_t B, int64_t S,
                          adnm_stream_t stream);
int64_t adnm_bridge_heads_bwd_ws_bytes(int64_t total, int64_t B, int64_t S);
int adnm_bridge_heads_bwd(const float* att, const float* const* W, const int64_t* C, int nheads, const float* enhance,
                          const float* threshold, const float* const* z, const float* const* dy, float* datt, float* const* dW,
                          float* const* dbias, float* denhance, float* dthreshold, void* ws, int64_t ws_bytes, int64_t B, int64_t S,
                          adnm_stream_t stream);

int64_t adnm_bridge_pool_ws_bytes(int64_t B, int64_t S);
int adnm_bridge_pool_fwd(int64_t n, const float* const* x, const int64_t* L, const int64_t* C, float* att, void* ws, int64_t ws_bytes, int64_t B,
                         adnm_stream_t stream);
int adnm_bridge_pool_bwd(int64_t n, const float* const* dxa, const float* datt, const int64_t* L, const int64_t* C, float* const* dx, int64_t B,
                         adnm_stream_t stream);

int64_t adnm_colsum_ws_bytes(int64_t rows, int64_t n);
int adnm_colsum(const float* x, float* out, int64_t rows, int64_t n, void* ws, int64_t ws_bytes, adnm_stream_t stream);

#define ADNM_SKGEMM_NT 0
#define ADNM_SKGEMM_NN 1
#define ADNM_SKGEMM_TN 2
int adnm_skgemm_supported(int op, int64_t M, int64_t N, int64_t K);
int64_t adnm_skgemm_ws_bytes(int op, int64_t M, int64_t N, int64_t K);
int adnm_skgemm(int op, const float* a, int64_t lda, const void* b, int64_t ldb, int b_dtype, const float* b_scale, const float* bias, float* c,
                int64_t ldc, float* dbias, void* ws, int64_t ws_bytes, void* slabs_uc, int64_t slabs_uc_bytes, int64_t M, int64_t N, int64_t K,
                int prec, float* q, adnm_stream_t stream);
int64_t adnm_skgemm_counter_bytes(int op, int64_t M, int64_t N, int64_t K);
void* adnm_uncached_alloc(int64_t bytes);
int adnm_uncached_free(void* ptr);

int64_t adnm_rainloss_ws_bytes(int64_t n);
int adnm_rainloss(const float* pred, const float* target, float* loss, float* grad, void* ws, int64_t ws_bytes, int64_t n, float omega_t,
                  float alpha, float gamma, adnm_stream_t stream);

int adnm_catmix_fwd(const void* x, int64_t ldx, const void* r, int64_t ldr, const void* f, int64_t ldf, const float* a1, const float* a2,
                    const float* a3, const float* a4, void* y, int64_t M, int64_t d, int dtype, adnm_stream_t stream);
int64_t adnm_catmix_bwd_ws_bytes(int64_t M, int64_t d);
int adnm_catmix_bwd(const void* dy, int64_t lddy, const void* x, int64_t ldx, const void* r, int64_t ldr, const void* f, int64_t ldf,
                    const float* a1, const float* a2, const float* a3, const float* a4, void* dx, void* dr, void* df, float* da, void* ws,
                    int64_t ws_bytes, int64_t M, int64_t d, int dtype, adnm_stream_t stream);

int adnm_lincomb_fwd(const void* x0, int64_t ld0, const void* x1, int64_t ld1, const void* x2, int64_t ld2,
                     const float* s0, const float* s1, const float* s2, const float* gamma, void* y, int64_t ldy,
                     int64_t M, int64_t C, int dtype, adnm_stream_t stream);
int64_t adnm_lincomb_bwd_ws_bytes(int64_t M, int64_t C);
int adnm_lincomb_bwd(const void* dy, int64_t lddy, const void* x0, int64_t ld0, const void* x1, int64_t ld1,
                     const void* x2, int64_t ld2, const float* s0, const float* s1, const float* s2,
                     const float* gamma, void* dx0, int64_t lddx0, void* dx1, int64_t lddx1, void* dx2, int64_t lddx2,
                     float* ds0, float* ds1, float* ds2, float* dgamma, void* ws, int64_t ws_bytes, int64_t M, int64_t C,
                     int dtype, adnm_stream_t stream);

int adnm_mixnorm_fwd(const float* x0, int64_t ld0, const float* x1, int64_t ld1, const float* s0, const float* s1, const float* gamma,
                     const float* w, const float* b, const float* scale, const float* shift, float* ymix, int64_t ldm, float* yn,
                     int64_t ldn, float* mu, float* rstd, int64_t M, int64_t d, float eps, int subtract_mean, adnm_stream_t stream);
int64_t adnm_mixnorm_bwd_ws_bytes(int64_t M, int64_t d);
int adnm_mixnorm_bwd(const float* dyn, int64_t lddyn, const float* dres, int64_t lddres, const float* x0, int64_t ld0, const float* x1,
                     int64_t ld1, const float* s0, const float* s1, const float* gamma, const float* w, const float* b, const float* scale,
                     const float* mu, const float* rstd, float* dx0, int64_t lddx0, float* dx1, int64_t lddx1, float* ds0, float* ds1,
                     float* dgamma, float* dw, float* db, float* dscale, float* dshift, void* ws, int64_t ws_bytes, int64_t M, int64_t d,
                     int subtract_mean, adnm_stream_t stream);

int64_t adnm_adamw_ws_bytes(void);
int adnm_adamw_step(float* p, const float* g, float* m, float* v, int64_t n, float* state, float lr, float beta1,
                    float beta2, float eps, float weight_decay, float max_norm, void* ws, int64_t ws_bytes, void* shadow, int shadow_dtype,
                    const int* seg_end, const int* seg_rec, int64_t nseg, float* wtab, const float* hyper, adnm_stream_t stream);
int adnm_shadow_refresh(const float* p, int64_t n, void* shadow, int shadow_dtype, const int* seg_end, const int* seg_rec, int64_t nseg,
                        float* wtab, int collect, adnm_stream_t stream);

int adnm_step_guard(const float* g, int64_t n, float* state, float max_norm, const float* hyper, void* ws, int64_t ws_bytes, void* stats,
                    adnm_stream_t stream);
int adnm_adamw_step_guarded(float* p, const float* g, float* m, float* v, int64_t n, float* state, float lr, float beta1, float beta2,
                            float eps, float weight_decay, float max_norm, void* shadow, int shadow_dtype, const int* seg_end,
                            const int* seg_rec, int64_t nseg, float* wtab, const float* hyper, const void* stats, adnm_stream_t stream);
int adnm_loss_stat(const float* loss, void* stats, adnm_stream_t stream);

int64_t adnm_conv3_ws_bytes(int64_t B, int64_t H, int64_t W, int64_t K, int64_t N);
int adnm_conv3_fwd(const float* in, int64_t ldin, const float* w, int64_t ws_n, int64_t ws_tap, int64_t ws_k, const float* bias,
                   float* out, int64_t ldo, float* pre, int64_t ldpre, void* ws, int64_t ws_bytes, int64_t B, int64_t H, int64_t W,
                   int64_t K, int64_t N, int act, int prec, float* q, adnm_stream_t stream);
int adnm_conv3_dgrad(const float* dout, int64_t lddo, const float* w, int64_t ws_n, int64_t ws_tap, int64_t ws_k, float* din,
                     int64_t lddin, void* ws, int64_t ws_bytes, int64_t B, int64_t H, int64_t W, int64_t K, int64_t N, int prec,
                     float* q, adnm_stream_t stream);
int64_t adnm_conv3_wgrad_ws_bytes(int64_t B, int64_t H, int64_t W, int64_t K, int64_t N);
int adnm_conv3_wgrad(const float* dout, int64_t lddo, const float* in, int64_t ldin, float* dw, float* dbias, void* ws,
                     int64_t ws_bytes, int64_t B, int64_t H, int64_t W, int64_t K, int64_t N, int prec, adnm_stream_t stream);

int adnm_convt_col2im(const float* cols, int64_t ldc, int64_t col_tap_stride, int64_t col_c_stride, const float* bias, float* out,
                      int64_t ldo, int64_t B, int64_t H, int64_t W, int64_t C, adnm_stream_t stream);
int adnm_convt_im2col(const float* dout, int64_t lddo, float* dcols, int64_t ldc, int64_t col_tap_stride, int64_t col_c_stride,
                      int64_t B, int64_t H, int64_t W, int64_t C, adnm_stream_t stream);

int adnm_radar_ingest(const void* src_u8, float* dst, int64_t frames, int64_t H0, int64_t W0, int64_t S, float mul, adnm_stream_t stream);
int adnm_batch_fetch(const float* store, int64_t n_samples, int64_t T, int64_t hw, const int32_t* order, int64_t order_len, int64_t pos,
                     float* x, float* tgt, int64_t B, int64_t T_in, adnm_stream_t stream);
int adnm_batch_fetch_aug(const float* store, int64_t n_samples, int64_t T, int64_t Hs, int64_t Ws, const int32_t* order, const int32_t* aug,
                         int64_t order_len, int64_t pos, float* x, float* tgt, int64_t B, int64_t T_in, int64_t H, int64_t W,
                         adnm_stream_t stream);
int64_t adnm_eval_counts_ws_bytes(int64_t frames, int64_t hw, int64_t nthr);
int adnm_eval_counts(const float* truth, const float* pred, float* out, const float* thresholds_host, int64_t nthr, float value_scale,
                     void* ws, int64_t ws_bytes, int64_t frames, int64_t hw, adnm_stream_t stream);
int64_t adnm_eval_ssim_ws_bytes(int64_t frames, int64_t H, int64_t W);
int adnm_eval_ssim(const float* truth, const float* pred, float* out, float value_scale, void* ws, int64_t ws_bytes, int64_t frames,
                   int64_t H, int64_t W, adnm_stream_t stream);

int64_t adnm_valid_block_bytes(int64_t T, int64_t nthr);
int64_t adnm_valid_accum_ws_bytes(int64_t frames, int64_t T, int64_t hw, int64_t nthr);
int adnm_valid_accum(const float* pred, const float* target, void* block, float* loss_out, const float* thresholds_host, int64_t nthr,
                     float value_scale, float omega_t, float alpha, float gamma, void* ws, int64_t ws_bytes, int64_t frames, int64_t T,
                     int64_t hw, adnm_stream_t stream);
int64_t adnm_valid_ssim_accum_ws_bytes(int64_t frames, int64_t T, int64_t H, int64_t W, int64_t nthr);
int adnm_valid_ssim_accum(const float* pred, const float* target, void* block, int64_t nthr, float value_scale, void* ws, int64_t ws_bytes,
                          int64_t frames, int64_t T, int64_t H, int64_t W, adnm_stream_t stream);

int64_t adnm_valid_pool_block_bytes(int64_t T, int64_t nthr, int64_t npool);
int64_t adnm_valid_pool_accum_ws_bytes(int64_t frames, int64_t T, int64_t H, int64_t W, int64_t nthr, const int64_t* pools_host, int64_t npool);
int adnm_valid_pool_accum(const float* pred, int64_t pred_sample_stride, int64_t pred_frame_stride, const float* target, void* table,
                          const float* thresholds_host, int64_t nthr, float value_scale, const int64_t* pools_host, int64_t npool, void* ws,
                          int64_t ws_bytes, int64_t frames, int64_t T, int64_t H, int64_t W, adnm_stream_t stream);

int64_t adnm_valid_fss_block_bytes(int64_t T, int64_t nthr, int64_t nscale);
int64_t adnm_valid_fss_accum_ws_bytes(int64_t frames, int64_t T, int64_t H, int64_t W, int64_t nthr, const int64_t* scales_host, int64_t nscale);
int adnm_valid_fss_accum(const float* pred, int64_t pred_sample_stride, int64_t pred_frame_stride, const float* target, void* table,
                         const float* thresholds_host, int64_t nthr, float value_scale, const int64_t* scales_host, int64_t nscale, void* ws,
                         int64_t ws_bytes, int64_t frames, int64_t T, int64_t H, int64_t W, adnm_stream_t stream);

int64_t adnm_trec_ws_bytes(int64_t samples, int64_t H, int64_t W, int64_t block, int64_t radius);
int adnm_trec_motion(const float* prev, const float* last, int64_t sample_stride, void* motion_i32, void* cost_out_u32_or_null, float value_scale,
                     int64_t block, int64_t radius, int64_t echo, void* ws, int64_t ws_bytes, int64_t samples, int64_t H, int64_t W,
                     adnm_stream_t stream);
int adnm_advect(const float* last, int64_t sample_stride, const void* motion_i32, float* out, int64_t block, int64_t samples, int64_t T, int64_t H,
                int64_t W, adnm_stream_t stream);

int64_t adnm_valid_spectrum_block_bytes(int64_t T, int64_t H, int64_t W);
int64_t adnm_valid_spectrum_accum_ws_bytes(int64_t frames, int64_t T, int64_t H, int64_t W);
int adnm_valid_spectrum_accum(const float* pred, int64_t pred_sample_stride, int64_t pred_frame_stride, const float* target, void* table,
                              float value_scale, void* ws, int64_t ws_bytes, int64_t frames, int64_t T, int64_t H, int64_t W,
                              adnm_stream_t stream);

int64_t adnm_valid_joint_levels(float value_scale);
int64_t adnm_valid_joint_block_bytes(int64_t T, float value_scale);
int64_t adnm_valid_joint_accum_ws_bytes(int64_t frames, int64_t T, int64_t hw, float value_scale);
int adnm_valid_joint_accum(const float* pred, int64_t pred_sample_stride, int64_t pred_frame_stride, const float* target, void* table,
                           float value_scale, void* ws, int64_t ws_bytes, int64_t frames, int64_t T, int64_t hw, adnm_stream_t stream);

int64_t adnm_valid_objects_block_bytes(int64_t T, int64_t nthr);
int64_t adnm_valid_objects_accum_ws_bytes(int64_t frames, int64_t T, int64_t H, int64_t W, int64_t nthr);
int adnm_valid_objects_accum(const float* pred, int64_t pred_sample_stride, int64_t pred_frame_stride, const float* target, void* table,
                             const float* thresholds_host, int64_t nthr, float value_scale, int64_t min_area, void* ws, int64_t ws_bytes,
                             int64_t frames, int64_t T, int64_t H, int64_t W, adnm_stream_t stream);
int64_t adnm_label_objects_ws_bytes(int64_t frames, int64_t T, int64_t H, int64_t W);
int adnm_label_objects(const float* src, int64_t sample_stride, int64_t frame_stride, void* labels_i32, float thr, float value_scale,
                       int64_t min_area, void* ws, int64_t ws_bytes, int64_t frames, int64_t T, int64_t H, int64_t W, adnm_stream_t stream);

int adnm_forecast_render(const float* pred, uint8_t* fields, uint8_t* strip, const float* bounds_host, const uint8_t* palette_host,
                         int64_t nbins, float pixel_scale, int64_t B, int64_t T, int64_t H, int64_t W, int64_t frame_start,
                         int64_t frame_step, int64_t gap, adnm_stream_t stream);

int adnm_act_fwd(const float* x, float* y, int64_t n, int act, adnm_stream_t stream);
int adnm_act_bwd(const float* dy, const float* pre, float* dpre, int64_t n, int act, adnm_stream_t stream);
int adnm_swish_fwd(const float* x, const float* beta, float* y, int64_t n, adnm_stream_t stream);
int64_t adnm_swish_bwd_ws_bytes(int64_t n);
int adnm_swish_bwd(const float* dy, const float* x, const float* beta, float* dx, float* dbeta, void* ws, int64_t ws_bytes, int64_t n,
                   adnm_stream_t stream);

int adnm_cast_f32_bf16(const void* src, void* dst, int64_t n, float scale, adnm_stream_t stream);
int adnm_cast_bf16_f32(const void* src, void* dst, int64_t n, float scale, adnm_stream_t stream);

int adnm_grad_accum(float* acc, const float* g, int64_t n, int first, adnm_stream_t stream);
int adnm_grad_accum_final(const float* acc, float* g, void* wire_bf16, int64_t n, float scale, adnm_stream_t stream);

int adnm_ema_update(const float* p, float* ema, int64_t n, const float* state, float decay, int warmup, float* info, const void* stats,
                    adnm_stream_t stream);
int adnm_ema_swap(float* p, float* ema, int64_t n, adnm_stream_t stream);

int adnm_tsgemm_supported(int64_t M, int64_t N, int64_t K);
int adnm_tsgemm_nt(const void* x, int64_t ldx, const float* w, int64_t ws_n, int64_t ws_k, const float* bias, void* y,
                   int64_t ldy, int64_t M, int64_t N, int64_t K, int prec, float* q, int x_dtype, int y_dtype, adnm_stream_t stream);
int adnm_tsgemm_tn_supported(int64_t M, int64_t N, int64_t K);
int64_t adnm_tsgemm_tn_ws_bytes(int64_t M, int64_t N, int64_t K);
int adnm_tsgemm_tn(const void* dy, int64_t lddy, const void* x, int64_t ldx, float* dw, float* dbias, void* ws,
                   int64_t ws_bytes, int64_t M, int64_t N, int64_t K, int dy_dtype, int x_dtype, adnm_stream_t stream);

int adnm_adnprep_fwd(float* const* params, float* const* prepped, int64_t d_model, int64_t d_inner, int64_t gn,
                     int64_t headdim, int64_t tap_ld, adnm_stream_t stream);
int64_t adnm_adnprep_bwd_ws_bytes(void);
int adnm_adnprep_bwd(float* const* params, float* const* gprepped, float* const* dparams, int64_t d_model,
                     int64_t d_inner, int64_t gn, int64_t headdim, int64_t tap_ld, void* ws, int64_t ws_bytes,
                     adnm_stream_t stream);
int adnm_wtprep_fwd(float* const* w, float* const* s, float* bias, float* const* taps, float* bias_t, int64_t C,
                    int64_t Cp, int64_t K, int64_t levels, adnm_stream_t stream);
int adnm_wtprep_bwd(float* const* w, float* const* s, float* bias, float* const* gtaps, float* gbias_t,
                    float* const* dw, float* const* ds, float* dbias, int64_t C, int64_t Cp, int64_t K, int64_t levels,
                    adnm_stream_t stream);
int adnm_adnprep_fwd_multi(int64_t n, float* const* params, float* const* prepped, const int64_t* dims, float* const* narrow, int narrow_dtype,
                           adnm_stream_t stream);
int64_t adnm_adnprep_bwd_multi_ws_bytes(int64_t n);
int adnm_adnprep_bwd_multi(int64_t n, float* const* params, float* const* gprepped, float* const* dparams, const int64_t* dims, void* ws,
                           int64_t ws_bytes, adnm_stream_t stream);
int adnm_wtprep_fwd_multi(int64_t n, float* const* w, float* const* s, float* const* bias, float* const* taps, float* const* bias_t,
                          const int64_t* dims, adnm_stream_t stream);
int adnm_wtprep_bwd_multi(int64_t n, float* const* w, float* const* s, float* const* bias, float* const* gtaps, float* const* gbias_t,
                          float* const* dw, float* const* ds, float* const* dbias, const int64_t* dims, adnm_stream_t stream);


#ifdef __cplusplus
}
#endif
#endif
```

Before: 531.8 sequences/s.

## Keep narrow bf16/fp8 weight shadows raw through staging instead of widening to fp32

The lgemm and skgemm kernels now hold bf16/fp8 weight-shadow operands in registers as packed raw words and build MFMA fragments or LDS tiles with byte permutes. Before, they were widened to fp32 and then repacked. A vectorized B-load path (16-byte bf16 / 8-byte fp8 per thread) is added for row-contiguous shadows when alignment allows. The skgemm prefetch ring is generalized to NB buffers, and the tuned-table lookup and workspace sizing become aware of the B dtype. This cuts conversion ALU work and register pressure on the weight side, at the cost of more template variants and a more complex plan lookup.

Result: no change. 535.7 sequences/s (median of 6 runs) (+0.7%).

```diff
diff --git a/adnm-unet_amd/csrc/adnm_common.h b/adnm-unet_amd/csrc/adnm_common.h
--- a/adnm-unet_amd/csrc/adnm_common.h
+++ b/adnm-unet_amd/csrc/adnm_common.h
@@ -195,6 +195,21 @@
   }
 }
 
+template <int BT>
+struct AdnmRawB {
+  using type = uint32_t;
+};
+template <>
+struct AdnmRawB<ADNM_B_BF16> {
+  using type = uint2;
+};
+template <int BT>
+__device__ __forceinline__ typename AdnmRawB<BT>::type adnm_ldb4_raw(const void* base, int64_t off) {
+  static_assert(BT == ADNM_B_BF16 || BT == ADNM_B_FP8, "raw loads are for the narrow shadows");
+  if constexpr (BT == ADNM_B_BF16) return *reinterpret_cast<const uint2*>(reinterpret_cast<const uint16_t*>(base) + off);
+  else return *reinterpret_cast<const uint32_t*>(reinterpret_cast<const uint8_t*>(base) + off);
+}
+
 using adnm_f32x4 = __attribute__((ext_vector_type(4))) float;
 using adnm_bf16x8 = __attribute__((ext_vector_type(8))) __bf16;
 
@@ -284,6 +299,36 @@
   } else {
 #pragma unroll
     for (int e = 0; e < 8; ++e) f.v[e] = t[e];
+  }
+  return f;
+}
+template <int PREC, bool HALF, typename Raw>
+__device__ __forceinline__ AdnmFrag<PREC> adnm_frag_raw(Raw lo, Raw hi) {
+  static_assert(PREC == ADNM_MFMA_BF16 || PREC == ADNM_MFMA_FP8, "raw fragments feed the narrow matrix-core modes");
+  AdnmFrag<PREC> f;
+  if constexpr (PREC == ADNM_MFMA_BF16) {
+    f.v = __builtin_bit_cast(adnm_bf16x8, make_uint4(lo.x, lo.y, HALF ? 0u : hi.x, HALF ? 0u : hi.y));
+  } else {
+    f.v = (long)(((unsigned long)(HALF ? 0u : hi) << 32) | (unsigned long)lo);
+  }
+  return f;
+}
+template <int PREC, bool HALF, typename Raw>
+__device__ __forceinline__ AdnmFrag<PREC> adnm_frag_raw_col(const Raw (&lo)[4], const Raw (&hi)[4], int b) {
+  static_assert(PREC == ADNM_MFMA_BF16 || PREC == ADNM_MFMA_FP8, "raw fragments feed the narrow matrix-core modes");
+  AdnmFrag<PREC> f;
+  if constexpr (PREC == ADNM_MFMA_BF16) {
+    const uint32_t sel = (b & 1) ? 0x07060302u : 0x05040100u;
+    auto src = [&](const Raw& w) { return b < 2 ? w.x : w.y; };
+    f.v = __builtin_bit_cast(adnm_bf16x8, make_uint4(__builtin_amdgcn_perm(src(lo[1]), src(lo[0]), sel), __builtin_amdgcn_perm(src(lo[3]), src(lo[2]), sel),
+                                                     HALF ? 0u : __builtin_amdgcn_perm(src(hi[1]), src(hi[0]), sel),
+                                                     HALF ? 0u : __builtin_amdgcn_perm(src(hi[3]), src(hi[2]), sel)));
+  } else {
+    const uint32_t sel = 0x0c0c0000u | ((4u + (uint32_t)b) << 8) | (uint32_t)b;
+    auto gather = [&](const Raw (&w)[4]) {
+      return __builtin_amdgcn_perm(__builtin_amdgcn_perm(w[3], w[2], sel), __builtin_amdgcn_perm(w[1], w[0], sel), 0x05040100u);
+    };
+    f.v = (long)(((unsigned long)(HALF ? 0u : gather(hi)) << 32) | (unsigned long)gather(lo));
   }
   return f;
 }
diff --git a/adnm-unet_amd/csrc/lgemm.hip b/adnm-unet_amd/csrc/lgemm.hip
--- a/adnm-unet_amd/csrc/lgemm.hip
+++ b/adnm-unet_amd/csrc/lgemm.hip
@@ -55,8 +55,22 @@
     return m.p[adnm_group_which(m, bid, nblk)];
   }
 };
-template <bool B_OC, int PREC, bool A_BF8, int D, int BT, bool MULTI>
+template <int BT>
+struct LgB {
+  float4 v[2];
+};
+template <>
+struct LgB<ADNM_B_BF16> {
+  uint32_t w[4];
+};
+template <>
+struct LgB<ADNM_B_FP8> {
+  uint32_t w[2];
+};
+
+template <bool B_OC, int PREC, bool A_BF8, int D, int BT, bool MULTI, bool BV = false>
 __global__ __launch_bounds__(kThreads) void lgemm_kernel(typename LgPick<MULTI>::Arg arg) {
+  static_assert(!BV || (BT != ADNM_B_F32 && !B_OC), "vector B loads: a narrow shadow contiguous along the reduction");
   int bid_ = 0, nblk_ = 0;
   const auto& p = LgPick<MULTI>::get(arg, &bid_, &nblk_);
   static_assert(BT == ADNM_B_F32 || (BT == ADNM_B_BF16 && PREC == ADNM_MFMA_BF16) || (BT == ADNM_B_FP8 && PREC == ADNM_MFMA_FP8),
@@ -95,7 +109,16 @@
       b_off[u] = (int)((jb + 4 <= p.J ? jb : p.J - 4) + (int64_t)(BF16 ? 2 * lr + u : lr + 16 * u) * p.ldb);
     }
   }
-  float4 ra[D][2], rb[D][2];
+  constexpr bool kRawB = BT != ADNM_B_F32;
+  const int vq = tid & 3, vrow = tid >> 2;
+  int bv_off = 0;
+  if constexpr (BV) {
+    const int jb = j0 + vrow;
+    bv_off = (int)((int64_t)(jb < p.J ? jb : p.J - 1) * p.ldb + 8 * vq);
+  }
+  float4 ra[D][2];
+  LgB<BT> rb[D];
+  auto bv_ok = [&](int kt) { return kt < nkt && (kt0 + kt) * kStep + 8 * vq < p.R; };
   auto a_ok = [&](int kt) { return kt < nkt && (kt0 + kt) * kStep + 4 * q < p.R; };
   auto b_ok = [&](int kt, int u) {
     if (!B_OC) return kt < nkt && (kt0 + kt) * kStep + 4 * q < p.R;
@@ -104,16 +127,33 @@
   int a_dead[2];
 #pragma unroll
   for (int u = 0; u < 2; ++u) a_dead[u] = (int)(p.A - a_row[u]);
-  auto load = [&](int kt, float4 (&av)[2], float4 (&bv)[2]) {
+  auto load = [&](int kt, float4 (&av)[2], LgB<BT>& bv) {
     const int r0 = (kt0 + kt) * kStep;
     const bool oka = a_ok(kt);
 #pragma unroll
     for (int u = 0; u < 2; ++u) {
       av[u] = *reinterpret_cast<const float4*>(a_row[u] + (oka ? r0 : a_dead[u]));
-      const int64_t bo = b_ok(kt, u) ? b_off[u] + (B_OC ? r0 * (int)p.ldb : r0) : 0;
-      if constexpr (BT == ADNM_B_FP8)
-        bv[u] = make_float4(__int_as_float(*reinterpret_cast<const int*>(reinterpret_cast<const uint8_t*>(p.B) + bo)), 0.f, 0.f, 0.f);
-      else bv[u] = adnm_ldb4<BT>(p.B, bo);
+      if constexpr (!BV) {
+        const int64_t bo = b_ok(kt, u) ? b_off[u] + (B_OC ? r0 * (int)p.ldb : r0) : 0;
+        if constexpr (BT == ADNM_B_BF16) {
+          const uint2 r = adnm_ldb4_raw<BT>(p.B, bo);
+          bv.w[2 * u] = r.x, bv.w[2 * u + 1] = r.y;
+        } else if constexpr (BT == ADNM_B_FP8) {
+          bv.w[u] = adnm_ldb4_raw<BT>(p.B, bo);
+        } else {
+          bv.v[u] = adnm_ldb4<BT>(p.B, bo);
+        }
+      }
+    }
+    if constexpr (BV) {
+      const int64_t bo = bv_ok(kt) ? bv_off + r0 : 0;
+      if constexpr (BT == ADNM_B_BF16) {
+        const uint4 r = *reinterpret_cast<const uint4*>(reinterpret_cast<const uint16_t*>(p.B) + bo);
+        bv.w[0] = r.x, bv.w[1] = r.y, bv.w[2] = r.z, bv.w[3] = r.w;
+      } else {
+        const uint2 r = *reinterpret_cast<const uint2*>(reinterpret_cast<const uint8_t*>(p.B) + bo);
+        bv.w[0] = r.x, bv.w[1] = r.y;
+      }
     }
   };
   float q_sa = 1.f, q_sb = 1.f, q_sbo = 1.f, amax_a = 0.f, amax_b = 0.f;
@@ -124,7 +164,41 @@
     rec_a = rec && (tile % p.tiles_j) == 0, rec_b = BT == ADNM_B_F32 && rec && (tile / p.tiles_j) == 0;
   }
   if (BT == ADNM_B_FP8) q_sb = 1.f, q_sbo = *p.b_scale;
-  auto stage = [&](int kt, int buf, const float4 (&av)[2], const float4 (&bv)[2]) {
+  auto stage_raw_b = [&](int kt, uint32_t* const sb, const LgB<BT>& bv) {
+    if constexpr (kRawB) {
+      constexpr int kW = BT == ADNM_B_BF16 ? 2 : 1;
+      if constexpr (BV) {
+        const bool ok = bv_ok(kt);
+        uint32_t* dst = sb + vrow * G::rc_stride + 2 * kW * vq;
+        if constexpr (BT == ADNM_B_BF16) *reinterpret_cast<uint4*>(dst) = make_uint4(ok ? bv.w[0] : 0u, ok ? bv.w[1] : 0u, ok ? bv.w[2] : 0u, ok ? bv.w[3] : 0u);
+        else *reinterpret_cast<uint2*>(dst) = make_uint2(ok ? bv.w[0] : 0u, ok ? bv.w[1] : 0u);
+      } else if constexpr (!B_OC) {
+#pragma unroll
+        for (int u = 0; u < 2; ++u) {
+          const bool ok = b_ok(kt, u);
+          uint32_t* dst = sb + (lrow + 32 * u) * G::rc_stride + kW * q;
+          if constexpr (BT == ADNM_B_BF16) *reinterpret_cast<uint2*>(dst) = make_uint2(ok ? bv.w[2 * u] : 0u, ok ? bv.w[2 * u + 1] : 0u);
+          else *dst = ok ? bv.w[u] : 0u;
+        }
+      } else if constexpr (BT == ADNM_B_BF16) {
+        const bool ok0 = b_ok(kt, 0), ok1 = b_ok(kt, 1);
+        const uint32_t e0 = ok0 ? bv.w[0] : 0u, e1 = ok0 ? bv.w[1] : 0u, o0 = ok1 ? bv.w[2] : 0u, o1 = ok1 ? bv.w[3] : 0u;
+        *reinterpret_cast<uint4*>(sb + lr * G::oc_stride + 4 * cq) =
+            make_uint4(__builtin_amdgcn_perm(o0, e0, 0x05040100u), __builtin_amdgcn_perm(o0, e0, 0x07060302u), __builtin_amdgcn_perm(o1, e1, 0x05040100u),
+                       __builtin_amdgcn_perm(o1, e1, 0x07060302u));
+      } else {
+        uint8_t* const sb8 = reinterpret_cast<uint8_t*>(sb);
+#pragma unroll
+        for (int u = 0; u < 2; ++u) {
+          const uint32_t w = b_ok(kt, u) ? bv.w[u] : 0u;
+          const int k = lr + 16 * u;
+#pragma unroll
+          for (int c = 0; c < 4; ++c) sb8[(4 * cq + c) * (4 * G::rc_stride) + k] = (uint8_t)(w >> (8 * c));
+        }
+      }
+    }
+  };
+  auto stage = [&](int kt, int buf, const float4 (&av)[2], const LgB<BT>& bvr) {
     uint32_t* const sa = ldsA + buf * kAW;
     uint32_t* const sb = ldsB + buf * kBW;
     const bool oka = a_ok(kt);
@@ -135,11 +209,13 @@
         amax_a = adnm_amax4(amax_a, v.x, v.y, v.z, v.w);
       }
     }
-    if (rec_b) {
-#pragma unroll
-      for (int u = 0; u < 2; ++u) {
-        const float4 v = keep_if(b_ok(kt, u), bv[u]);
-        amax_b = adnm_amax4(amax_b, v.x, v.y, v.z, v.w);
+    if constexpr (!kRawB) {
+      if (rec_b) {
+#pragma unroll
+        for (int u = 0; u < 2; ++u) {
+          const float4 v = keep_if(b_ok(kt, u), bvr.v[u]);
+          amax_b = adnm_amax4(amax_b, v.x, v.y, v.z, v.w);
+        }
       }
     }
     if constexpr (FP8) {
@@ -155,17 +231,20 @@
       };
 #pragma unroll
       for (int u = 0; u < 2; ++u) sa[(lrow + 32 * u) * G::rc_stride + q] = q4(keep_if(oka, av[u]), q_sa, A_BF8);
-#pragma unroll
-      for (int u = 0; u < 2; ++u) {
-        const float4 v = keep_if(b_ok(kt, u), bv[u]);
-        const uint32_t w = BT == ADNM_B_FP8 ? (uint32_t)__float_as_int(v.x) : q4(v, q_sb, false);
-        if (!B_OC) {
-          sb[(lrow + 32 * u) * G::rc_stride + q] = w;
-        } else {
-          uint8_t* const sb8 = reinterpret_cast<uint8_t*>(sb);
-          const int k = lr + 16 * u;
-#pragma unroll
-          for (int c = 0; c < 4; ++c) sb8[(4 * cq + c) * (4 * G::rc_stride) + k] = (uint8_t)(w >> (8 * c));
+      if constexpr (kRawB) {
+        stage_raw_b(kt, sb, bvr);
+      } else {
+#pragma unroll
+        for (int u = 0; u < 2; ++u) {
+          const uint32_t w = q4(keep_if(b_ok(kt, u), bvr.v[u]), q_sb, false);
+          if (!B_OC) {
+            sb[(lrow + 32 * u) * G::rc_stride + q] = w;
+          } else {
+            uint8_t* const sb8 = reinterpret_cast<uint8_t*>(sb);
+            const int k = lr + 16 * u;
+#pragma unroll
+            for (int c = 0; c < 4; ++c) sb8[(4 * cq + c) * (4 * G::rc_stride) + k] = (uint8_t)(w >> (8 * c));
+          }
         }
       }
       return;
@@ -177,20 +256,22 @@
       if (BF16) *reinterpret_cast<uint2*>(dst + 2 * q) = make_uint2(pack2(v.x, v.y), pack2(v.z, v.w));
       else *reinterpret_cast<float4*>(dst + 4 * q) = v;
     }
-    if (!B_OC) {
+    if constexpr (kRawB) {
+      stage_raw_b(kt, sb, bvr);
+    } else if (!B_OC) {
 #pragma unroll
       for (int u = 0; u < 2; ++u) {
-        const float4 v = keep_if(b_ok(kt, u), bv[u]);
+        const float4 v = keep_if(b_ok(kt, u), bvr.v[u]);
         uint32_t* dst = sb + (lrow + 32 * u) * G::rc_stride;
         if (BF16) *reinterpret_cast<uint2*>(dst + 2 * q) = make_uint2(pack2(v.x, v.y), pack2(v.z, v.w));
         else *reinterpret_cast<float4*>(dst + 4 * q) = v;
       }
     } else if (BF16) {
-      const float4 v0 = keep_if(b_ok(kt, 0), bv[0]), v1 = keep_if(b_ok(kt, 1), bv[1]);
+      const float4 v0 = keep_if(b_ok(kt, 0), bvr.v[0]), v1 = keep_if(b_ok(kt, 1), bvr.v[1]);
       *reinterpret_cast<uint4*>(sb + lr * G::oc_stride + 4 * cq) = make_uint4(pack2(v0.x, v1.x), pack2(v0.y, v1.y), pack2(v0.z, v1.z), pack2(v0.w, v1.w));
     } else {
 #pragma unroll
-      for (int u = 0; u < 2; ++u) *reinterpret_cast<float4*>(sb + (lr + 16 * u) * G::oc_stride + 4 * cq) = keep_if(b_ok(kt, u), bv[u]);
+      for (int u = 0; u < 2; ++u) *reinterpret_cast<float4*>(sb + (lr + 16 * u) * G::oc_stride + 4 * cq) = keep_if(b_ok(kt, u), bvr.v[u]);
     }
   };
 
@@ -370,17 +451,17 @@
 
 constexpr int kRingDepth = 4;
 
-template <bool B_OC, int PREC, bool A_BF8, int BT>
+template <bool B_OC, int PREC, bool A_BF8, int BT, bool BV = false>
 int lg_group_fn(const AdnmGroupRec* const* r, int n, hipStream_t st) {
   if (n == 1) {
     LgArgs p;
     memcpy(&p, r[0]->args, sizeof(LgArgs));
-    lgemm_kernel<B_OC, PREC, A_BF8, kRingDepth, BT, false><<<(unsigned)r[0]->grid, kThreads, 0, st>>>(p);
+    lgemm_kernel<B_OC, PREC, A_BF8, kRingDepth, BT, false, BV><<<(unsigned)r[0]->grid, kThreads, 0, st>>>(p);
     return ADNM_OK;
   }
   AdnmMulti<LgArgs> m;
   const unsigned blocks = adnm_group_pack(r, n, m);
-  lgemm_kernel<B_OC, PREC, A_BF8, kRingDepth, BT, true><<<blocks, kThreads, 0, st>>>(m);
+  lgemm_kernel<B_OC, PREC, A_BF8, kRingDepth, BT, true, BV><<<blocks, kThreads, 0, st>>>(m);
   return ADNM_OK;
 }
 
@@ -435,9 +516,14 @@
   AdnmGroupRec rec;
   rec.grid = pl.ntiles * pl.nbs, rec.pos = 0, rec.prof = prof, rec.bytes = prof_bytes;
   memcpy(rec.args, &p, sizeof(LgArgs));
+  const int64_t esz = b_dtype == ADNM_B_BF16 ? 2 : 1;
+  const bool bv = !b_oc && b_dtype != ADNM_B_F32 && (uintptr_t)b % (8 * esz) == 0 && ldb % 8 == 0 && R % 8 == 0;
 #define LG(OC)                                                                                              \
   do {                                                                                                      \
-    if (b_dtype == ADNM_B_BF16) rec.fn = lg_group_fn<OC, ADNM_MFMA_BF16, false, ADNM_B_BF16>;               \
+    if (!OC && bv && b_dtype == ADNM_B_BF16) rec.fn = lg_group_fn<false, ADNM_MFMA_BF16, false, ADNM_B_BF16, true>; \
+    else if (!OC && bv && prec == ADNM_MFMA_FP8) rec.fn = lg_group_fn<false, ADNM_MFMA_FP8, false, ADNM_B_FP8, true>; \
+    else if (!OC && bv) rec.fn = lg_group_fn<false, ADNM_MFMA_FP8, true, ADNM_B_FP8, true>;                 \
+    else if (b_dtype == ADNM_B_BF16) rec.fn = lg_group_fn<OC, ADNM_MFMA_BF16, false, ADNM_B_BF16>;          \
     else if (b_dtype == ADNM_B_FP8 && prec == ADNM_MFMA_FP8) rec.fn = lg_group_fn<OC, ADNM_MFMA_FP8, false, ADNM_B_FP8>; \
     else if (b_dtype == ADNM_B_FP8) rec.fn = lg_group_fn<OC, ADNM_MFMA_FP8, true, ADNM_B_FP8>;              \
     else if (prec == ADNM_MFMA_BF16) rec.fn = lg_group_fn<OC, ADNM_MFMA_BF16, false, ADNM_B_F32>;           \
diff --git a/adnm-unet_amd/csrc/skgemm.hip b/adnm-unet_amd/csrc/skgemm.hip
--- a/adnm-unet_amd/csrc/skgemm.hip
+++ b/adnm-unet_amd/csrc/skgemm.hip
@@ -26,7 +26,20 @@
   AdnmQuant* q;
 };
 
-template <bool A_RC, bool B_RC, int PREC, bool A_BF8, int TM, int TN, int KC, int BT = ADNM_B_F32, typename Args>
+template <int BT, bool B_RC, int TN, int KC>
+struct SkB {
+  typename AdnmRawB<BT>::type w[KC][B_RC ? TN : 4];
+};
+template <bool B_RC, int TN, int KC>
+struct SkB<ADNM_B_F32, B_RC, TN, KC> {
+  float v[TN][KC][4];
+};
+template <int TM, int KC>
+struct SkA {
+  float v[TM][KC][4];
+};
+
+template <bool A_RC, bool B_RC, int PREC, bool A_BF8, int TM, int TN, int KC, int BT = ADNM_B_F32, int NB = 3, typename Args>
 __device__ __forceinline__ void skgemm_body(const Args& p, const int bid, const int nblk) {
   static_assert(BT == ADNM_B_F32 || (BT == ADNM_B_BF16 && PREC == ADNM_MFMA_BF16) || (BT == ADNM_B_FP8 && PREC == ADNM_MFMA_FP8),
                 "a narrow weight shadow feeds the matrix-core precision it was made for");
@@ -50,7 +63,11 @@
   const int c0 = active ? (bslice * p.wpt + gw) * p.chunks_per_wave : 0;
   const int c1 = !active ? 0 : (c0 + p.chunks_per_wave < p.nchunks ? c0 + p.chunks_per_wave : p.nchunks);
 
-  auto fetch = [&](int c, bool live, float (&av)[TM][KC][4], float (&bv)[TN][KC][4]) {
+  using ABuf = SkA<TM, KC>;
+  using BBuf = SkB<BT, B_RC, TN, KC>;
+  constexpr bool kRawB = BT != ADNM_B_F32;
+  auto fetch = [&](int c, bool live, ABuf& abuf, BBuf& bbuf) {
+    auto& av = abuf.v;
 #pragma unroll
     for (int s = 0; s < KC; ++s) {
       const int r0 = (c * KC + s) * 16;
@@ -75,16 +92,26 @@
 #pragma unroll
         for (int t = 0; t < TN; ++t) {
           const int col = j0 + 16 * t + l15, cc = col < p.J ? col : p.J - 1;
-          const float4 v = adnm_ldb4<BT>(p.B, live ? (int64_t)cc * p.sb_j + rq4 : 0);
-          bv[t][s][0] = v.x, bv[t][s][1] = v.y, bv[t][s][2] = v.z, bv[t][s][3] = v.w;
+          const int64_t off = live ? (int64_t)cc * p.sb_j + rq4 : 0;
+          if constexpr (kRawB) {
+            bbuf.w[s][t] = adnm_ldb4_raw<BT>(p.B, off);
+          } else {
+            const float4 v = adnm_ldb4<BT>(p.B, off);
+            bbuf.v[t][s][0] = v.x, bbuf.v[t][s][1] = v.y, bbuf.v[t][s][2] = v.z, bbuf.v[t][s][3] = v.w;
+          }
         }
       } else {
         const int col = j0 + 4 * l15, cc = col < p.J ? col : p.J - 4;
 #pragma unroll
         for (int e = 0; e < 4; ++e) {
           const int rr = r0 + 4 * kk + e, rq = rr < p.R ? rr : p.R - 1;
-          const float4 v = adnm_ldb4<BT>(p.B, live ? (int64_t)rq * p.sb_r + cc : 0);
-          bv[0][s][e] = v.x, bv[1 % TN][s][e] = v.y, bv[2 % TN][s][e] = v.z, bv[3 % TN][s][e] = v.w;
+          const int64_t off = live ? (int64_t)rq * p.sb_r + cc : 0;
+          if constexpr (kRawB) {
+            bbuf.w[s][e] = adnm_ldb4_raw<BT>(p.B, off);
+          } else {
+            const float4 v = adnm_ldb4<BT>(p.B, off);
+            bbuf.v[0][s][e] = v.x, bbuf.v[1 % TN][s][e] = v.y, bbuf.v[2 % TN][s][e] = v.z, bbuf.v[3 % TN][s][e] = v.w;
+          }
         }
       }
     }
@@ -104,7 +131,8 @@
     rec_a = rec && (tile % p.tiles_j) == 0, rec_b = BT == ADNM_B_F32 && rec && (tile / p.tiles_j) == 0;
   }
   if (BT == ADNM_B_FP8) q_sb = 1.f, q_sbo = *p.b_scale;
-  auto compute = [&](int c, float (&av)[TM][KC][4], const float (&bv)[TN][KC][4]) {
+  auto compute = [&](int c, ABuf& abuf, const BBuf& bbuf) {
+    auto& av = abuf.v;
 #pragma unroll
     for (int s = 0; s < KC; ++s) {
       const int r0 = (c * KC + s) * 16;
@@ -124,9 +152,11 @@
 #pragma unroll
         for (int t = 0; t < TM; ++t) amax_a = adnm_amax4(amax_a, av[t][s][0], av[t][s][1], av[t][s][2], av[t][s][3]);
       }
-      if (rec_b && r0 + 16 <= p.R) {
-#pragma unroll
-        for (int t = 0; t < TN; ++t) amax_b = adnm_amax4(amax_b, bv[t][s][0], bv[t][s][1], bv[t][s][2], bv[t][s][3]);
+      if constexpr (!kRawB) {
+        if (rec_b && r0 + 16 <= p.R) {
+#pragma unroll
+          for (int t = 0; t < TN; ++t) amax_b = adnm_amax4(amax_b, bbuf.v[t][s][0], bbuf.v[t][s][1], bbuf.v[t][s][2], bbuf.v[t][s][3]);
+        }
       }
     }
 #pragma unroll
@@ -136,7 +166,11 @@
 #pragma unroll
       for (int a = 0; a < TM; ++a) fa[a] = adnm_make_frag<PREC, A_BF8>(av[a][s], kHalf ? nullptr : av[a][(s + 1) % KC], q_sa);
 #pragma unroll
-      for (int b = 0; b < TN; ++b) fb[b] = adnm_make_frag<PREC, false>(bv[b][s], kHalf ? nullptr : bv[b][(s + 1) % KC], q_sb);
+      for (int b = 0; b < TN; ++b) {
+        if constexpr (!kRawB) fb[b] = adnm_make_frag<PREC, false>(bbuf.v[b][s], kHalf ? nullptr : bbuf.v[b][(s + 1) % KC], q_sb);
+        else if constexpr (B_RC) fb[b] = adnm_frag_raw<PREC, kHalf>(bbuf.w[s][b], bbuf.w[(s + 1) % KC][b]);
+        else fb[b] = adnm_frag_raw_col<PREC, kHalf>(bbuf.w[s], bbuf.w[(s + 1) % KC], b);
+      }
 #pragma unroll
       for (int a = 0; a < TM; ++a)
 #pragma unroll
@@ -146,26 +180,23 @@
         }
     }
   };
-  float a0[TM][KC][4], b0[TN][KC][4], a1[TM][KC][4], b1[TN][KC][4], a2[TM][KC][4], b2[TN][KC][4];
+  ABuf ra[NB];
+  BBuf rb[NB];
   const int cl = c1 > c0 ? c1 - 1 : 0;
-  auto fetch_at = [&](int c, float (&av)[TM][KC][4], float (&bv)[TN][KC][4]) { fetch(c < c1 ? c : cl, c < c1, av, bv); };
-  fetch_at(c0, a0, b0);
-  __builtin_amdgcn_sched_barrier(0);
-  fetch_at(c0 + 1, a1, b1);
-  __builtin_amdgcn_sched_barrier(0);
-  for (int c = c0; c < c1; c += 3) {
-    fetch_at(c + 2, a2, b2);
+  auto fetch_at = [&](int c, ABuf& av, BBuf& bv) { fetch(c < c1 ? c : cl, c < c1, av, bv); };
+#pragma unroll
+  for (int s = 0; s < NB - 1; ++s) {
+    fetch_at(c0 + s, ra[s], rb[s]);
     __builtin_amdgcn_sched_barrier(0);
-    compute(c, a0, b0);
-    __builtin_amdgcn_sched_barrier(0);
-    fetch_at(c + 3, a0, b0);
-    __builtin_amdgcn_sched_barrier(0);
-    if (c + 1 < c1) compute(c + 1, a1, b1);
-    __builtin_amdgcn_sched_barrier(0);
-    fetch_at(c + 4, a1, b1);
-    __builtin_amdgcn_sched_barrier(0);
-    if (c + 2 < c1) compute(c + 2, a2, b2);
-    __builtin_amdgcn_sched_barrier(0);
+  }
+  for (int c = c0; c < c1; c += NB) {
+#pragma unroll
+    for (int s = 0; s < NB; ++s) {
+      fetch_at(c + s + NB - 1, ra[(s + NB - 1) % NB], rb[(s + NB - 1) % NB]);
+      __builtin_amdgcn_sched_barrier(0);
+      if (s == 0 || c + s < c1) compute(c + s, ra[s], rb[s]);
+      __builtin_amdgcn_sched_barrier(0);
+    }
   }
 
   if (rec_a) adnm_amax_commit(&p.q->amax_a, amax_a);
@@ -377,21 +408,26 @@
 struct Tuned {
   int op, I, J, R, bf16;
   int cfg[6];
+  int bt = ADNM_B_F32;
 };
 const Tuned kTuned[] = {
 #include "skgemm_tuned.inc"
 };
-const Tuned* tuned(int op, int64_t I, int64_t J, int64_t R, bool bf16) {
+const Tuned* tuned(int op, int64_t I, int64_t J, int64_t R, bool bf16, int bt) {
+  const Tuned* wide = nullptr;
   for (const Tuned& t : kTuned)
-    if (t.op == op && t.I == I && t.J == J && t.R == R && t.bf16 == (int)bf16) return &t;
-  return nullptr;
+    if (t.op == op && t.I == I && t.J == J && t.R == R && t.bf16 == (int)bf16) {
+      if (t.bt == bt) return &t;
+      if (t.bt == ADNM_B_F32) wide = &t;
+    }
+  return wide;
 }
 Plan plan_deferred(int64_t I, int64_t J, int64_t R, bool direct, bool bf16) {
   Plan pl;
   pl.kernel = KERNEL_STREAM, pl.combine = false, pl.tm = pl.tn = 4, pl.kc = 1;
   finish(pl, I, J, R);
   const bool force = forced().on;
-  const Tuned* tu = force || use_table() == 0 ? nullptr : tuned(ADNM_SKGEMM_TN, I, J, R, bf16);
+  const Tuned* tu = force || use_table() == 0 ? nullptr : tuned(ADNM_SKGEMM_TN, I, J, R, bf16, ADNM_B_F32);
   if (force || tu) {
     const int* v = force ? forced().v : tu->cfg;
     pl.wpt = v[4], pl.nbs = v[5];
@@ -422,11 +458,11 @@
   slice(pl);
   return pl;
 }
-Plan plan_critical(int op, int64_t I, int64_t J, int64_t R, bool can_split, bool bf16) {
+Plan plan_critical(int op, int64_t I, int64_t J, int64_t R, bool can_split, bool bf16, int bt) {
   Plan pl;
   pl.combine = false;
   const bool force = forced().on;
-  const Tuned* tu = force || use_table() == 0 ? nullptr : tuned(op, I, J, R, bf16);
+  const Tuned* tu = force || use_table() == 0 ? nullptr : tuned(op, I, J, R, bf16, bt);
   if (force || tu) {
     const int* v = force ? forced().v : tu->cfg;
     pl.kernel = v[0], pl.tm = v[1], pl.tn = v[2], pl.kc = v[3], pl.wpt = v[4], pl.nbs = v[5];
@@ -459,8 +495,13 @@
   pl.combine = pl.nbs > 1;
   return pl;
 }
-Plan make_plan(int op, int64_t I, int64_t J, int64_t R, bool direct, bool bf16) {
-  return op == ADNM_SKGEMM_TN ? plan_deferred(I, J, R, direct, bf16) : plan_critical(op, I, J, R, !direct && J % 4 == 0, bf16);
+Plan make_plan(int op, int64_t I, int64_t J, int64_t R, bool direct, bool bf16, int bt) {
+  return op == ADNM_SKGEMM_TN ? plan_deferred(I, J, R, direct, bf16) : plan_critical(op, I, J, R, !direct && J % 4 == 0, bf16, bt);
+}
+template <typename F>
+void for_each_plan(int op, int64_t I, int64_t J, int64_t R, F&& f) {
+  f(make_plan(op, I, J, R, false, false, ADNM_B_F32));
+  for (int bt : {ADNM_B_F32, ADNM_B_BF16, ADNM_B_FP8}) f(make_plan(op, I, J, R, false, true, bt));
 }
 
 }
@@ -521,10 +562,22 @@
 
 extern "C" int64_t adnm_skgemm_ws_bytes(int op, int64_t M, int64_t N, int64_t K) {
   if (!shape_ok(op, M, N, K)) return -1;
+  int64_t I, J, R, need = 0;
+  dims(op, M, N, K, &I, &J, &R);
+  for_each_plan(op, I, J, R, [&](const Plan& pl) {
+    const int64_t n = ws_need(pl, I, J, R);
+    if (n > need) need = n;
+  });
+  return need;
+}
+
+extern "C" int64_t adnm_skgemm_plan_ws_bytes(int op, int64_t M, int64_t N, int64_t K, int prec, int b_dtype) {
+  if (!shape_ok(op, M, N, K) || prec < ADNM_MFMA_F32 || prec > ADNM_MFMA_FP8_GRAD) return -1;
+  const bool fp8 = prec == ADNM_MFMA_FP8 || prec == ADNM_MFMA_FP8_GRAD;
+  if (!(b_dtype == ADNM_B_F32 || (op != ADNM_SKGEMM_TN && ((b_dtype == ADNM_B_BF16 && prec == ADNM_MFMA_BF16) || (b_dtype == ADNM_B_FP8 && fp8))))) return -1;
   int64_t I, J, R;
   dims(op, M, N, K, &I, &J, &R);
-  const int64_t a = ws_need(make_plan(op, I, J, R, false, false), I, J, R), b = ws_need(make_plan(op, I, J, R, false, true), I, J, R);
-  return a > b ? a : b;
+  return ws_need(make_plan(op, I, J, R, false, prec != ADNM_MFMA_F32, b_dtype), I, J, R);
 }
 
 extern "C" int64_t adnm_skgemm_counter_bytes(int op, int64_t M, int64_t N, int64_t K) {
@@ -532,16 +585,15 @@
   if (op == ADNM_SKGEMM_TN) return 0;
   int64_t I, J, R, need = 0;
   dims(op, M, N, K, &I, &J, &R);
-  for (int bf = 0; bf < 2; ++bf) {
-    const Plan pl = make_plan(op, I, J, R, false, bf != 0);
-    if (pl.kernel < 0) continue;
+  for_each_plan(op, I, J, R, [&](const Plan& pl) {
+    if (pl.kernel < 0) return;
     int64_t ntiles = pl.ntiles, nbs = pl.nbs;
     if (pl.kernel == KERNEL_LDS) {
       ntiles = adnm_cdiv(I, 64) * adnm_cdiv(J, 64);
       nbs = adnm_lgemm_ws_bytes(I, J, R, pl.nbs) > 16 ? 2 : 1;
     }
     if (nbs > 1 && adnm_ticket_bytes(ntiles) > need) need = adnm_ticket_bytes(ntiles);
-  }
+  });
   return need;
 }
 
@@ -566,8 +618,8 @@
                "skgemm: operands must be aligned to 4 elements (16 bytes of fp32)");
   hipStream_t st = (hipStream_t)stream;
   const bool bf = prec != ADNM_MFMA_F32;
-  Plan pl = make_plan(op, I, J, R, false, bf);
-  if (op == ADNM_SKGEMM_TN && ldc != J) pl = make_plan(op, I, J, R, true, bf);
+  Plan pl = make_plan(op, I, J, R, false, bf, b_dtype);
+  if (op == ADNM_SKGEMM_TN && ldc != J) pl = make_plan(op, I, J, R, true, bf, b_dtype);
   ADNM_REQUIRE(pl.kernel >= 0, "skgemm: ADNM_SK_FORCE names a configuration this op has no kernel for");
   if (!(slabs_uc && op != ADNM_SKGEMM_TN)) {
     const int64_t asked = adnm_skgemm_ws_bytes(op, M, N, K);
diff --git a/include/adnm_hip.h b/include/adnm_hip.h
--- a/include/adnm_hip.h
+++ b/include/adnm_hip.h
@@ -187,6 +187,7 @@
                 int64_t ldc, float* dbias, void* ws, int64_t ws_bytes, void* slabs_uc, int64_t slabs_uc_bytes, int64_t M, int64_t N, int64_t K,
                 int prec, float* q, adnm_stream_t stream);
 int64_t adnm_skgemm_counter_bytes(int op, int64_t M, int64_t N, int64_t K);
+int64_t adnm_skgemm_plan_ws_bytes(int op, int64_t M, int64_t N, int64_t K, int prec, int b_dtype);
 void* adnm_uncached_alloc(int64_t bytes);
 int adnm_uncached_free(void* ptr);
 
```
